# mit-acl/dpgo

Hardware: AMD Instinct MI355X
Metric: rbcd_iterations_per_sec (higher is better)
Workload: dtype f64; 1 GPU; synthetic 3-D grid 50x50x40 (100000 poses, 293500 edges), init = perturbed truth; agents=1, agents_per_gpu=1, r=5, d=3, schedule=single agent, poses_per_agent=100000, nnzb_per_agent=687000

## Files before the change

### dpgo_amd/csrc/agents.hip

```cpp
#include "host.h"

namespace dpgo_host {

int rebuild_vals(dpgo_problem_s* p, int nnzb, const int32_t* cptr, const int32_t* cedge, const uint8_t* ckind,
                 const double* base, double sign, double* out) {
  if (nnzb <= 0) return DPGO_OK;
  const int g = std::max(1, std::min(kMaxGrid, (nnzb + kBlock - 1) / kBlock));
  if (p->d == 2)
    launch(k_rebuild_Q<2>, g, 0, p->stream, p->gnc.dev(), cptr, cedge, ckind, base, sign, out, nnzb);
  else
    launch(k_rebuild_Q<3>, g, 0, p->stream, p->gnc.dev(), cptr, cedge, ckind, base, sign, out, nnzb);
  HIPC(hipGetLastError());
  return DPGO_OK;
}
int rebuild_Q_from_weights(dpgo_problem_s* p, const double* base, double sign, double* out) {
  return rebuild_vals(p, p->Q.nnzb, p->gnc.c_ptr, p->gnc.c_edge, p->gnc.c_kind, base, sign, out);
}
int rebuild_C_from_weights(dpgo_problem_s* p, const double* base, double sign, double* out) {
  if (!p->gnc.g_ptr) return DPGO_OK;
  return rebuild_vals(p, p->C.nnzb, p->gnc.g_ptr, p->gnc.g_edge, p->gnc.g_kind, base, sign, out);
}
int refresh_after_weights(dpgo_problem_s* p) {
  CHK(rebuild_Q_from_weights(p, p->gnc.q_base, 1.0, p->Q.vals));
  CHK(rebuild_C_from_weights(p, p->gnc.c_base, 1.0, p->C.vals));
// ... 633 lines not shown
  }
  HIPC(hipGetLastError());
  return DPGO_OK;
}
}
int dpgo_flags_wait_device(int n, unsigned long long* const* words_dev, const unsigned long long* values, int timeout_ms,
                           void* stream) {
  if (n < 0 || (n > 0 && (!words_dev || !values)) || timeout_ms <= 0) return fail(DPGO_ERR_INVALID, "bad ordering-word arguments");
  return flags_wait(n, words_dev, values, timeout_ms, nullptr, stream);
}
int dpgo_flags_wait_device_checked(int n, unsigned long long* const* words_dev, const unsigned long long* values,
                                   long long timeout_ms, unsigned long long* err_word, void* stream) {
  if (n < 0 || (n > 0 && (!words_dev || !values)) || timeout_ms < 0 || (timeout_ms > 0 && !err_word))
    return fail(DPGO_ERR_INVALID, "bad ordering-word arguments");
  return flags_wait(n, words_dev, values, timeout_ms, err_word, stream);
}

int dpgo_exchange_plan_destroy(dpgo_exchange_plan_t pl) {
  delete pl;
  return DPGO_OK;
}


int dpgo_max_translation_distance_device(int r, int d, int n, const double* X_dev, const double* Xprev_dev,
                                         double* out_dev, double* out_host, void* stream) {
  if (!X_dev || !Xprev_dev || !out_dev || n <= 0) return fail(DPGO_ERR_INVALID, "bad arguments");
  hipStream_t s = (hipStream_t)stream;
  HIPC(hipMemsetAsync(out_dev, 0, sizeof(double), s));
  const int g = std::max(1, std::min(kMaxGrid, (n + kBlock - 1) / kBlock));
  CHK(dispatch_dr(d, r, [&](auto D, auto R) {
    return launch(k_max_translation_distance<D, R>, g, 0, s, X_dev, Xprev_dev, n,
                  reinterpret_cast<unsigned long long*>(out_dev));
  }));
  HIPC(hipGetLastError());
  if (out_host) {
    HIPC(hipMemcpyAsync(out_host, out_dev, sizeof(double), hipMemcpyDeviceToHost, s));
    HIPC(hipStreamSynchronize(s));
  }
  return DPGO_OK;
}


int dpgo_manifold_project(int r, int d, int n, const double* M, double* out, int device) {
  if (!M || !out) return fail(DPGO_ERR_INVALID, "null pointer");
  CHK(manifold_args(r, d, n, device));
  const size_t total = (size_t)n * (d + 1) * r, vb = sizeof(double) * total;
  DevBuf<double> a, o;
  CHK(a.alloc(total));
  CHK(o.alloc(total));
  HIPC(hipMemcpy(a, M, vb, hipMemcpyHostToDevice));
  CHK(dpgo_manifold_project_device(r, d, n, a, o, nullptr));
  HIPC(hipMemcpy(out, o, vb, hipMemcpyDeviceToHost));
  return DPGO_OK;
}


int dpgo_manifold_tangent_project(int r, int d, int n, const double* X, const double* V, double* out, int device) {
  if (!X || !V || !out) return fail(DPGO_ERR_INVALID, "null pointer");
  CHK(manifold_args(r, d, n, device));
  const size_t total = (size_t)n * (d + 1) * r, vb = sizeof(double) * total;
  DevBuf<double> x, v, o;
  for (DevBuf<double>* q : {&x, &v, &o}) CHK(q->alloc(total));
  HIPC(hipMemcpy(x, X, vb, hipMemcpyHostToDevice));
  HIPC(hipMemcpy(v, V, vb, hipMemcpyHostToDevice));
  CHK(dispatch_dr(d, r, [&](auto D, auto R) {
    return launch(k_precond<D, R>, tiles_grid(d, n), 0, nullptr, x, v, nullptr, o, n);
  }));
  HIPC(hipGetLastError());
  HIPC(hipMemcpy(out, o, vb, hipMemcpyDeviceToHost));
  return DPGO_OK;
}


int dpgo_manifold_retract(int r, int d, int n, const double* X, const double* eta, double scale, double* out,
                          int device) {
  if (!X || !eta || !out) return fail(DPGO_ERR_INVALID, "null pointer");
  CHK(manifold_args(r, d, n, device));
  const size_t total = (size_t)n * (d + 1) * r, vb = sizeof(double) * total;
  DevBuf<double> x, v, o;
  for (DevBuf<double>* q : {&x, &v, &o}) CHK(q->alloc(total));
  HIPC(hipMemcpy(x, X, vb, hipMemcpyHostToDevice));
  HIPC(hipMemcpy(v, eta, vb, hipMemcpyHostToDevice));
  CHK(dispatch_dr(d, r, [&](auto D, auto R) {
    return launch(k_retract<D, R>, tiles_grid(d, n), 0, nullptr, x, v, scale, o, nullptr, n, nullptr, nullptr, nullptr);
  }));
  HIPC(hipGetLastError());
  HIPC(hipMemcpy(out, o, vb, hipMemcpyDeviceToHost));
  return DPGO_OK;
}

}
```

### dpgo_amd/csrc/host.h

```cpp
#pragma once
#include "kernels.h"

#include <algorithm>
#include <atomic>
#include <chrono>
#include <condition_variable>
#include <functional>
#include <memory>
#include <pthread.h>
#include <sched.h>
#include <mutex>
#include <thread>
#include <type_traits>
#include <cmath>
#include <cstdio>
#include <cstdlib>
#include <cstring>
#include <string>
#include <utility>
#include <vector>

#include "../../include/dpgo_hip.h"

using namespace dpgo;
// ... 76 lines not shown

template <class T, bool kPinned>
class OwnedBuf {
 public:
  OwnedBuf() = default;
  OwnedBuf(OwnedBuf&& o) noexcept : p_(std::exchange(o.p_, nullptr)), bytes_(std::exchange(o.bytes_, 0)) {}
  OwnedBuf& operator=(OwnedBuf&& o) noexcept {
    if (this != &o) {
      reset();
      p_ = std::exchange(o.p_, nullptr);
      bytes_ = std::exchange(o.bytes_, 0);
    }
    return *this;
  }
  ~OwnedBuf() { reset(); }
  int alloc(size_t count, unsigned flags = hipHostMallocDefault) {
    reset();
    const size_t bytes = sizeof(T) * count;
    if constexpr (kPinned)
      HIPC(hipHostMalloc(&p_, bytes, flags));
    else
      HIPC(hipMalloc(&p_, bytes));
    if (!p_) return DPGO_OK;
    bytes_ = bytes;
    g_live_buffers.fetch_add(1, std::memory_order_relaxed);
    g_live_bytes.fetch_add((long long)bytes, std::memory_order_relaxed);
    return DPGO_OK;
  }
  void reset() {
    if (!p_) return;
    if constexpr (kPinned)
      (void)hipHostFree(p_);
    else
      (void)hipFree(p_);
    g_live_buffers.fetch_sub(1, std::memory_order_relaxed);
    g_live_bytes.fetch_sub((long long)bytes_, std::memory_order_relaxed);
    p_ = nullptr;
    bytes_ = 0;
  }
  T* get() const { return p_; }
  operator T*() const { return p_; }
  T* operator->() const { return p_; }

 private:
  T* p_ = nullptr;
  size_t bytes_ = 0;
};
template <class T>
using DevBuf = OwnedBuf<T, false>;
template <class T>
using PinBuf = OwnedBuf<T, true>;

template <class T>
inline int upload(DevBuf<T>& dst, const T* src, size_t count, hipStream_t s) {
  CHK(dst.alloc(count > 0 ? count : 1));
  if (count > 0) HIPC(hipMemcpyAsync(dst, src, sizeof(T) * count, hipMemcpyHostToDevice, s));
  return DPGO_OK;
}

struct OwnedStream {
  hipStream_t s = nullptr;
  OwnedStream() = default;
  OwnedStream(const OwnedStream&) = delete;
  OwnedStream& operator=(const OwnedStream&) = delete;
  ~OwnedStream() {
    if (s) (void)hipStreamDestroy(s);
  }
  operator hipStream_t() const { return s; }
};

struct Bsr {
  int nrows = 0, ncols = 0, nnzb = 0;
  DevBuf<int32_t> rowptr, colidx;
  DevBuf<double> vals;
  BsrDev dev() const { return BsrDev{rowptr, colidx, vals}; }
};

#define DPGO_OPTIONS(X)                                                                                                  \
  X(split,             "DPGO_SPLIT",              0,  "lane groups per pose of the SpMM-family kernels: 1, 2, 4 (0: by size)")       \
  X(spmm_symmetric,    "DPGO_SPMM_SYMMETRIC",    -1,  "symmetric storage of Q for blocks beyond the Infinity Cache: 0 / 1")          \
  X(stream_nt,         "DPGO_STREAM_NT",         -1,  "non-temporal single-use operands in the tCG-step kernels: 0 / 1")             \
  X(outer_sym,         "DPGO_OUTER_SYM",          1,  "outer RTR iteration (k_grad / k_hess) reads the symmetric copy when tCG does") \
  X(rho_exact,         "DPGO_RHO_EXACT",          0,  "rho test from a fresh H eta (k_hess, one more pass over Q) instead of tCG's residual: reference path") \
  X(tile_walk,         "DPGO_TILE_WALK",          1,  "symmetric-storage kernels walk each XCD's tiles breadth-first over the tile graph (0: index order)") \
  X(tcg_ahead,         "DPGO_TCG_AHEAD",          0,  "iterations the just-in-time feed stays ahead (0: 2 multilevel / 4 otherwise)") \
  X(grid_update,       "DPGO_GRID_UPDATE",        0,  "launch cap of k_tcg_update (0: resident count)")                              \
  X(grid_hess,         "DPGO_GRID_HESS",          0,  "launch cap of k_tcg_hess (0: resident count)")                                \
  X(grid_hess_sym,     "DPGO_GRID_HESS_SYM",      0,  "launch cap of k_tcg_hess_sym (0: resident count)")                            \
  X(grid_retract,      "DPGO_GRID_RETRACT",       0,  "launch cap of k_retract (0: 1024)")                                           \
  X(grid_outer_sym,    "DPGO_GRID_OUTER_SYM",     0,  "launch cap of k_grad / k_hess on the symmetric storage (0: resident count)")  \
  X(grid_spmm_sym,     "DPGO_GRID_SPMM_SYM",      0,  "launch cap of k_spmm_sym (0: resident count, at most 1024)")                  \
  X(grid_ml,           "DPGO_GRID_ML",            0,  "launch cap of the level-0 restriction / post-smoothing (0: resident count)")  \
  X(grid_edges,        "DPGO_GRID_EDGES",         0,  "launch cap of k_edge_robust, GNC and robust re-weighting alike (0: 1024)")    \
  X(persist,           "DPGO_PERSIST",           -1,  "one-launch solve (k_rtr_persist) off / on whatever the size: 0 / 1")          \
  X(persist_max_poses, "DPGO_PERSIST_MAX_POSES",  0,  "largest block the one-launch solve takes (0: every block it can hold)")       \
  X(persist_split,     "DPGO_PERSIST_SPLIT",      0,  "lane groups per pose of the one-launch solve: 1, 4 (0: by size)")             \
  X(persist_mt,        "DPGO_PERSIST_MT",         0,  "tiles per workgroup of the one-launch solve: 1, 2 (0: by size)")              \
  X(additive_tiles,    "DPGO_ADDITIVE_TILES",     1,  "workgroup tiles per aggregate of the additive one-launch solve: 1, 2 (opt-in: blocks up to ~28 000 poses)") \
  X(poll_first,        "DPGO_POLL_FIRST",        -1,  "s_sleep units before the first sweep of the in-kernel all-reduce")            \
  X(poll_sleep,        "DPGO_POLL_SLEEP",        -1,  "s_sleep units between sweeps of the in-kernel all-reduce")                    \
  X(poll_first_pay,    "DPGO_POLL_FIRST_PAY",    -1,  "the same before the first sweep of a reduction that carries a payload")       \
  X(persist_verbose,   "DPGO_PERSIST_VERBOSE",    0,  "per-solve phase report of the one-launch solve on stderr")                    \
  X(setup_timing,      "DPGO_SETUP_TIMING",       0,  "section times of the hierarchy's symbolic set-up on stderr")                  \
  X(setup_threads,     "DPGO_SETUP_THREADS",      0,  "host threads of the hierarchy's symbolic set-up (0: min(8, cores); 1: serial)") \
  X(setup_pin,         "DPGO_SETUP_PIN",          1,  "set-up worker threads placed in the CPU group of the thread that first used them") \
  X(auto_cost_rule,    "DPGO_AUTO_COST_RULE",     1,  "DPGO_PRECOND_AUTO on coupled blocks: cost rule (0: tCG-budget hysteresis only)") \
  X(ml_graph,          "DPGO_ML_GRAPH",           1,  "graph aggregates in the default hierarchy (0: index runs)")                   \
  X(ml_graph_size,     "DPGO_ML_GRAPH_SIZE",      0,  "growth size of the default graph aggregates (0: by size)")                    \
  X(ml_growth_chunks,  "DPGO_ML_GROWTH_CHUNKS",   0,  "index ranges the graph aggregates grow and merge in (0: 8 from 65 536 poses, else 1)") \
  X(ml_ap,             "DPGO_ML_AP",              1,  "two-level post-smoothing through A P (0: gather through Q; index runs only)") \
  X(ml_dense_sym,      "DPGO_ML_DENSE_SYM",      -1,  "dense level from the packed lower triangle on the matrix cores: 0 / 1")       \
  X(ml_early_stop,     "DPGO_ML_EARLY_STOP",      1,  "tCG's residual test in the restriction kernel, one kernel early")             \
  X(ml_operator_bits,  "DPGO_ML_OPERATOR_BITS",   0,  "level-0 operator copies of the cycle on HBM-bound blocks: 32 / 64 (0: 32)")   \
  X(ml_vector_bits,    "DPGO_ML_VECTOR_BITS",     0,  "cycle-internal vectors (pre-smoothed iterate, kept residual) beside fp32 operator copies: 32 / 64 (0: 32)") \
  X(ml_dense_bits,     "DPGO_ML_DENSE_BITS",      0,  "dense level beside fp32 cycle vectors: 32 / 64 (0: 64 -- fp32 measured neutral)") \
  X(gj_mfma,           "DPGO_GJ_MFMA",            1,  "rank-64 updates of the dense inverse on the fp64 matrix cores")               \
  X(dense_chunk,       "DPGO_DENSE_CHUNK",        0,  "tiles per workgroup of k_dense_sym_apply (0: default)")                       \
  X(coarse_nodes,      "DPGO_COARSE_NODES",       0,  "nodes per workgroup of k_ml_coarse_prolong: 1-4 (0: by size)")                \
  X(coarse_grid,       "DPGO_COARSE_GRID",        0,  "launch cap of k_ml_coarse_prolong (0: default)")                              \
  X(coarse_nt,         "DPGO_COARSE_NT",         -1,  "non-temporal loads of the dense inverse: 0 / 1")
struct Options {
#define X(field, var, unset, text) int field = unset;
  DPGO_OPTIONS(X)
#undef X
};
inline Options& options_storage() {
  static Options o;
  return o;
}
inline void options_read(Options& o) {
  o = Options();
#define X(field, var, unset, text) \
  if (const char* e_ = std::getenv(var)) o.field = (*e_ == 0) ? 1 : std::atoi(e_);
  DPGO_OPTIONS(X)
#undef X
}
inline const Options& options() {
  static const bool once = (options_read(options_storage()), true);
  (void)once;
  return options_storage();
}
inline std::string options_describe() {
  const Options& o = options();
  std::string s;
#define X(field, var, unset, text) s += std::string(var) + "=" + std::to_string(o.field) + (o.field == (unset) ? "" : " [set]") + "  # " + text + "\n";
  DPGO_OPTIONS(X)
#undef X
  return s;
}

}
using namespace dpgo_host;

struct dpgo_problem_s {
  int r = 0, d = 0, n = 0, b = 0, T = 0;
  int device = 0;
  OwnedStream own_stream;
  hipStream_t stream = nullptr;
  Bsr Q;
  Bsr C;
  DevBuf<double> G0, G;
  bool has_G = false;
  DevBuf<double> dinv;
  double dinv_shift = -1.0;
  DevBuf<double> x1_buf, x2, g1, g2, eta, delta, Hd, rr, z, S1, S2;
  double* x1 = nullptr;
  struct MlLevel {
    int n = 0;
    int k = 0;
    int split = 1;
    Bsr A;
    DevBuf<int32_t> slot_row;
    DevBuf<double> dinv, Pb;
    DevBuf<double> r, x1, x;
    Bsr AP;
    DevBuf<double> res1;
    bool graph = false;
    DevBuf<int32_t> lab, agg_ptr, agg_mem, parent, pslot;
    DevBuf<int32_t> mem_pos;
    DevBuf<int32_t> seg_info, seg_ptr;
    int nseg = 0;
    DevBuf<int32_t> tile_perm;
    int perm_tile = 0;
    int merge_cap = 0;
    DevBuf<double> tbuf;
    DevBuf<float> Pb32, AP32;
    DevBuf<float> x1f, res1f;
    AggMap agg() const { return AggMap{graph ? lab : nullptr, k}; }
  };
  std::vector<MlLevel> ml;
  std::vector<int32_t> h_rowptr, h_colidx;
  bool ml_symbolic = false, ml_ready = false, ml_user_ks = false;
  bool ml_additive_layout = false;
  struct AddPlan {
    int split = 0, tile = 0, S = 0, cap = 0, na = 0;
    bool graph = true;
  } add_plan;
  bool add_plan_known = false;
  int add_tiles = 0;
  struct AggCache {
    int S = 0, cap = 0;
    std::vector<int32_t> lab, ptr, mem, parent, pslot;
  } add_agg;
  double ml_omega = 0.7, ml_shift = 1e-1;
  struct DenseLevel {
    DevBuf<double> inv;
    DevBuf<float> inv32;
    DevBuf<double> packed, pd, pt;
    DevBuf<DenseChunk> chunks;
    DevBuf<int> chunk_first;
    int nchunks = 0;
    int lda = 0;
    DevBuf<double> W, Rx;
  } dense;
  bool ml_use_dense_sym() const {
    const int env = options().ml_dense_sym;
    if (!ml_use_ap() || ml_coarse_bits != 64 || !dense.packed || env == 0) return false;
    return env == 1 || dense.lda >= 3072;
  }
  int ml_coarse_bits = 64;
  int ml_operator_bits = 32;
  bool ml_ops32_ready = false;
  bool ml_ops32_suspend = false;
  bool ml_ops32_wanted() const { return ml_operator_bits == 32 && tcg_sym && split == 1 && ml_use_ap() && sym.uvalsT != nullptr; }
  bool ml_ops32_active() const { return !ml_ops32_suspend && ml_ops32_wanted() && ml_ops32_ready; }
  bool ml_vec32_active() const { return ml_ops32_active() && options().ml_vector_bits != 64; }
  bool coarse32_active() const {
    return ml_coarse_bits == 32 || (ml_vec32_active() && !ml_use_dense_sym() && options().ml_dense_bits == 32);
  }
  bool auto_ml = false, auto_decided = false;
  struct AutoCost {
    long long jac_units = 0;
    int ref = 0;
    int state = 0;
    int backoff = 0;
    int switches = 0;
    int last_used = -1, last_products = 0;
    int uj = 10, ua = 18;
  } auto_cost;
  void auto_decide() {
    if (!auto_decided) {
      auto_ml = !(has_G || C.nnzb > 0);
      auto_decided = true;
      auto_cost = AutoCost();
    }
  }
  bool ml_use_ap() const {
    const bool off = options().ml_ap == 0;
    return ml.size() == 2 && ml[0].AP.vals != nullptr && (!off || ml[0].graph);
// ... 161 lines not shown
    wait(submit(count, fn, max_threads));
  }
  void warm(int threads) {
    bool expected = false;
    if (threads <= 1 || !warmed_.compare_exchange_strong(expected, true)) return;
    std::thread([this, threads] { wait(submit(threads - 1, [](int) {}, threads)); }).detach();
  }

 private:
  static constexpr int kMaxWorkers = 15;
  int home_cpu_ = -1;
  void pin(int) {
    if (!pin_enabled() || home_cpu_ < 0) return;
    cpu_set_t allowed, want;
    CPU_ZERO(&allowed);
    CPU_ZERO(&want);
    if (sched_getaffinity(0, sizeof(allowed), &allowed) != 0) return;
    const int lo = home_cpu_ & ~7;
    int cnt = 0;
    for (int c = lo; c < lo + 8; ++c)
      if (c < CPU_SETSIZE && CPU_ISSET(c, &allowed)) CPU_SET(c, &want), ++cnt;
    if (cnt >= 2) (void)pthread_setaffinity_np(pthread_self(), sizeof(want), &want);
  }
  static bool pin_enabled() { return options().setup_pin != 0; }
  TaskPool() { home_cpu_ = sched_getcpu(); }
  static void help(Batch& b) {
    for (;;) {
      const int k = b.next.fetch_add(1, std::memory_order_relaxed);
      if (k >= b.count) return;
      b.fn(k);
      b.done.fetch_add(1, std::memory_order_release);
    }
  }
  void loop() {
    for (;;) {
      Job b;
      {
        std::unique_lock<std::mutex> lk(mu_);
        cv_.wait(lk, [this] { return !queue_.empty(); });
        b = std::move(queue_.front());
        queue_.erase(queue_.begin());
      }
      help(*b);
    }
  }
  std::mutex mu_;
  std::condition_variable cv_;
  std::vector<Job> queue_;
  unsigned nworkers_ = 0;
  std::atomic<bool> warmed_{false};
};
struct JobGuard {
  TaskPool::Job job;
  ~JobGuard() { TaskPool::get().wait(job); }
};

struct PersistGeo {
  int split = 0, mt = 0, wgs = 0, slots = 0;
};

enum { RUN_FULL = 0, RUN_BEGIN = 1, RUN_END = 2 };

int set_device(dpgo_problem_s* p);
int upload_bsr(Bsr& m, int nrows, int ncols, int nnzb, int b, const int32_t* rowptr, const int32_t* colidx,
               const double* vals, hipStream_t s);
int validate_bsr(int nrows, int ncols, int nnzb, const int32_t* rowptr, const int32_t* colidx, bool need_diag);
int build_dinv(dpgo_problem_s* p, double shift);
int poll_state(dpgo_problem_s* p);
int push_state(dpgo_problem_s* p);
void sym_free(dpgo_problem_s* p);
int launch_spmm_view(dpgo_problem_s* p, const BsrDev& M, const double* V, const double* Gadd, double* OUT, int rows, int g,
                     bool stream_nt = false);
int sym_symbolic_setup(dpgo_problem_s* p);
int sym_ensure(dpgo_problem_s* p, bool* usable);
int launch_spmm_sym(dpgo_problem_s* p, const BsrSymDev& M, const double* V, const double* Gadd, double* OUT);
int launch_spmm(dpgo_problem_s* p, const Bsr& M, const double* V, const double* Gadd, double* OUT, int nrows = -1,
                bool plain_only = false);
bool outer_sym_enabled();
int launch_grad(dpgo_problem_s* p, const double* X, double* RG, double* S, double* EG,
                const DevState* st = nullptr, bool sym = false);
int launch_hess(dpgo_problem_s* p, const double* X, const double* S, const double* V, const double* Gdot,
                double* HV, double* partials, const DevState* st, int check_tcg, bool sym = false);
int launch_retract(dpgo_problem_s* p, const double* X, const double* eta, double scale, double* X2,
                   const DevState* st, const double* rho_r = nullptr, const double* rho_g = nullptr);
int launch_rtr_update(dpgo_problem_s* p);
int launch_precond(dpgo_problem_s* p, const double* X, const double* V, const double* dinv, double* Z);
int launch_rtr_begin(dpgo_problem_s* p, double tol, double Delta0, double Dmax, int max_inner, int tiny);
int check_ready(dpgo_problem_s* p);
int h2d(dpgo_problem_s* p, double* dst, const double* src);
int d2h(dpgo_problem_s* p, double* dst, const double* src);

int ml_tile(int b, int split);
int additive_tile(const dpgo_problem_s* p);
int ml_level_split(int n);
int ml_default_graph_size(int n, int b);
std::vector<int> ml_default_ks(int n, int b, int split0);
void ml_free(dpgo_problem_s* p);
int ml_graph_aggregates(const std::vector<int32_t>& rowptr, const std::vector<int32_t>& colidx, int n, int S,
                        std::vector<int32_t>& lab, std::vector<int32_t>& ptr, std::vector<int32_t>& mem,
                        std::vector<int32_t>& parent, std::vector<int32_t>& pslot);
int ml_merge_small_aggregates(const std::vector<int32_t>& rowptr, const std::vector<int32_t>& colidx, int n, int S, int cap,
                              std::vector<int32_t>& lab, std::vector<int32_t>& ptr, std::vector<int32_t>& mem,
                              std::vector<int32_t>& parent, std::vector<int32_t>& pslot);
int ml_symbolic_setup(dpgo_problem_s* p, const std::vector<int>& ks_in, int perm_tile = 0);
int setup_threads();
int flat_grid(size_t items);
bool gj_use_mfma();
int dense_spd_inverse(hipStream_t s, double* M, int lda, double* W, double* Rx, bool mfma);
int ml_numeric_setup(dpgo_problem_s* p);
std::vector<int> ml_current_ks(const dpgo_problem_s* p);
const dpgo_problem_s::AddPlan& additive_plan(dpgo_problem_s* p);
int additive_split_of(const dpgo_problem_s* p);
int additive_tiles(const dpgo_problem_s* p);
int additive_mt_of(const dpgo_problem_s* p);
int ml_ensure(dpgo_problem_s* p, double shift, bool additive = false);
int ml_ops32_ensure(dpgo_problem_s* p);
int persist_capacity(int device);
int launch_coarse_prolong(dpgo_problem_s* p, const dpgo_problem_s::MlLevel& L, const dpgo_problem_s::MlLevel& C,
                          const DevState* gate, double* xc_out = nullptr);
int launch_dense_sym(dpgo_problem_s* p, const dpgo_problem_s::MlLevel& C, const DevState* gate);
int launch_ml_restrict0(dpgo_problem_s* p, const double* r, const DevState* gate, int g0, bool stop_check = false);
int launch_ml_post_ap(dpgo_problem_s* p, const double* Xdev, const double* r, double* z, double* pout, const DevState* gate);
int launch_ml_tail(dpgo_problem_s* p, const double* Xdev, const double* r, double* z, double* pout,
                   const DevState* gate, bool stop_check = false);
int launch_ml_apply(dpgo_problem_s* p, const double* Xdev, const double* v, double* z);

int launch_tcg_update(dpgo_problem_s* p, const double* dinv, int first, double* z_out = nullptr,
                      double ml_omega = 0.0);
int launch_tcg_hess(dpgo_problem_s* p, int first);
int launch_tcg_hess_with(dpgo_problem_s* p, const DevState* sin, DevState* sout, int first, unsigned long long* hflag,
                         unsigned gen);
int resolve_tcg_storage(dpgo_problem_s* p);
int persist_capacity(int device);
bool persist_reserve(dpgo_problem_s* p, int slots, int limit);
void persist_release(dpgo_problem_s* p);
bool additive_available(dpgo_problem_s* p);
PersistGeo persist_geometry(const dpgo_problem_s* p, int free_slots, int share = 1, bool additive = false);
bool additive_lds_fits(const dpgo_problem_s* p, int split, int mt, int na);
int launch_rtr_persistent(dpgo_problem_s* p, const dpgo_ropt_params* prm, const double* dinv, bool* used, bool additive);
void persist_report(dpgo_problem_s* p);
int rtr_outer_iteration(dpgo_problem_s* p, const dpgo_ropt_params* prm, const double* dinv, Counters& cnt,
                        bool poll_at_end);
int auto_units_jacobi(dpgo_problem_s* p);
int auto_units_additive(dpgo_problem_s* p);
void auto_update(dpgo_problem_s* p, const dpgo_ropt_params* prm, int used, int products);
int run_optimize(dpgo_problem_s* p, const dpgo_ropt_params* prm, dpgo_ropt_result* res, int phase = RUN_FULL);
int tune_launch_caps(dpgo_problem_s* p);
int tune_persist(dpgo_problem_s* p);

int rebuild_vals(dpgo_problem_s* p, int nnzb, const int32_t* cptr, const int32_t* cedge, const uint8_t* ckind,
                 const double* base, double sign, double* out);
int rebuild_Q_from_weights(dpgo_problem_s* p, const double* base, double sign, double* out);
int rebuild_C_from_weights(dpgo_problem_s* p, const double* base, double sign, double* out);
int refresh_after_weights(dpgo_problem_s* p);

}
```

### dpgo_amd/csrc/kernels/manifold.h

```cpp
#pragma once

template <int D, int R>
__global__ __launch_bounds__(kBlock) void k_precond(const double* __restrict__ X, const double* __restrict__ V,
                                                    const double* __restrict__ dinv, double* __restrict__ Z,
                                                    int n) {
  using GEO = Geo<D, R>;
  __shared__ double sm[kWaves][3][GEO::G][GEO::T];
  const LaneId L = lane_id<D>();
  const int ntiles = (n + GEO::P - 1) / GEO::P;
  const TileIter ti_ = tile_iter(ntiles);
  for (int tile = ti_.first; tile < ti_.last; tile += ti_.step) {
    const int i = tile * GEO::P + L.wave * GEO::G + L.g;
    const bool ok = (L.g < GEO::G) && (i < n);
    const size_t off = (size_t)i * GEO::T + L.c * R;
    double* ys = ok ? &sm[L.wave][0][L.g][0] : nullptr;
    double* vs = ok ? &sm[L.wave][1][L.g][0] : nullptr;
    double* zs = ok ? &sm[L.wave][2][L.g][0] : nullptr;
    double v[R], x[R], z[R];
    if (ok) {
      load_col<R>(X + off, x);
      load_col<R>(V + off, v);
      store_col<R>(ys + L.c * R, x);
      store_col<R>(vs + L.c * R, v);
    }
    wave_sync();
    if (ok) {
      if (dinv) {
        jacobi_col<D, R>(vs, dinv + (size_t)i * GEO::BB + L.c * GEO::B, z);
      } else {
#pragma unroll
        for (int a = 0; a < R; ++a) z[a] = v[a];
      }
      store_col<R>(zs + L.c * R, z);
    }
    wave_sync();
    if (ok) {
      double out[R], s[D];
      proj_col<D, R>(ys, zs, L.c, z, out, s);
      store_col<R>(Z + off, out);
    }
    wave_sync();
  }
}

template <int D, int R, bool RHO = false>
__global__ __launch_bounds__(kBlock) void k_retract(const double* __restrict__ X, const double* __restrict__ eta,
                                                    double scale, double* __restrict__ X2,
                                                    const DevState* __restrict__ st, int n,
                                                    const double* __restrict__ r, const double* __restrict__ g,
                                                    double* __restrict__ partials) {
  using GEO = Geo<D, R>;
  __shared__ double sm[kWaves][GEO::G][GEO::T];
  __shared__ double red[kWaves * kNP];
  if (st && st->rtr_stop) return;
  const LaneId L = lane_id<D>();
  const int ntiles = (n + GEO::P - 1) / GEO::P;
  [[maybe_unused]] double part[2] = {0.0, 0.0};
  const TileIter ti_ = tile_iter(ntiles);
  for (int tile = ti_.first; tile < ti_.last; tile += ti_.step) {
    const int i = tile * GEO::P + L.wave * GEO::G + L.g;
    const bool ok = (L.g < GEO::G) && (i < n);
    const size_t off = (size_t)i * GEO::T + L.c * R;
    double* as = ok ? &sm[L.wave][L.g][0] : nullptr;
    double a[R];
    if (ok) {
      double x[R], e[R];
      load_col<R>(X + off, x);
      load_col<R>(eta + off, e);
      if constexpr (RHO) {
        double rc[R], gc[R];
        load_col<R>(r + off, rc);
        load_col<R>(g + off, gc);
#pragma unroll
        for (int k = 0; k < R; ++k) {
          part[0] = fma(e[k], rc[k] - gc[k], part[0]);
          part[1] = fma(e[k], gc[k], part[1]);
        }
      }
#pragma unroll
      for (int k = 0; k < R; ++k) a[k] = fma(scale, e[k], x[k]);
      store_col<R>(as + L.c * R, a);
    }
    wave_sync();
    if (ok) {
      qf_col<D, R>(as, L.c, a);
      store_col<R>(X2 + off, a);
    }
    wave_sync();
  }
  if constexpr (RHO) store_partials<2>(part, partials, red);
}

constexpr double kJacobiTol = 0x1p-50;
constexpr double kJacobiZero = 0x1p-600;
constexpr int kJacobiSweeps = 30;
template <int D, int N>
__device__ __forceinline__ void jacobi_columns(double (&a)[D][N], double (&V)[D][D]) {
  double mx = 0.0;
#pragma unroll
  for (int p = 0; p < D; ++p)
#pragma unroll
    for (int k = 0; k < N; ++k) mx = fmax(mx, fabs(a[p][k]));
  const int ex = (mx > 0.0 && mx < INFINITY) ? -ilogb(mx) : 0;
#pragma unroll
  for (int p = 0; p < D; ++p) {
#pragma unroll
    for (int k = 0; k < N; ++k) a[p][k] = ldexp(a[p][k], ex);
#pragma unroll
    for (int q = 0; q < D; ++q) V[p][q] = (p == q) ? 1.0 : 0.0;
  }
  for (int sweep = 0; sweep < kJacobiSweeps; ++sweep) {
    bool rotated = false;
#pragma unroll
    for (int p = 0; p < D; ++p)
#pragma unroll
      for (int q = p + 1; q < D; ++q) {
        double al = 0.0, be = 0.0, ga = 0.0;
#pragma unroll
        for (int k = 0; k < N; ++k) {
          al = fma(a[p][k], a[p][k], al);
          be = fma(a[q][k], a[q][k], be);
          ga = fma(a[p][k], a[q][k], ga);
        }
        if (al > kJacobiZero && be > kJacobiZero && fabs(ga) > kJacobiTol * (sqrt(al) * sqrt(be))) {
          rotated = true;
          const double zeta = (be - al) / (2.0 * ga);
          const double t = (zeta >= 0.0 ? 1.0 : -1.0) / (fabs(zeta) + sqrt(zeta * zeta + 1.0));
          const double cs = 1.0 / sqrt(t * t + 1.0), sn = t * cs;
#pragma unroll
          for (int k = 0; k < N; ++k) {
            const double x = a[p][k], y = a[q][k];
            a[p][k] = cs * x - sn * y;
            a[q][k] = sn * x + cs * y;
          }
#pragma unroll
          for (int k = 0; k < D; ++k) {
            const double x = V[k][p], y = V[k][q];
            V[k][p] = cs * x - sn * y;
            V[k][q] = sn * x + cs * y;
          }
        }
      }
    if (!rotated) break;
  }
}
template <int D, int N>
__device__ __forceinline__ void jacobi_inv_norms(const double (&a)[D][N], double (&nrm2)[D], double (&inv)[D]) {
#pragma unroll
  for (int p = 0; p < D; ++p) {
    double s = 0.0;
#pragma unroll
// ... 143 lines not shown
```

### dpgo_amd/csrc/kernels/tcg.h

```cpp
#pragma once

__device__ __forceinline__ bool tcg_hess_prologue(DevState& st, const double* __restrict__ pin, int nb_in, int first,
                                                  double* red, double& beta, const PartialRaw<2>* early = nullptr) {
  double pr[2];
  if (early)
    partials_finish<2>(*early, pr, red);
  else
    load_partials<2>(pin, nb_in, pr, red);
  const double r_r = pr[0], z_r_new = pr[1];
  beta = 0.0;
  if (first) {
    st.norm_r0 = sqrt(r_r);
    st.z_r = z_r_new;
    st.d_Pd = z_r_new;
    st.e_Pd = 0.0;
    if (st.max_inner <= 0) {
      st.tcg_done = 1;
      return false;
    }
    return true;
  }
  const double norm_r = sqrt(r_r);
  const double pw = (st.theta == 1.0) ? st.norm_r0 : pow(st.norm_r0, st.theta);
  if (st.tcg_j >= st.min_inner && norm_r <= st.norm_r0 * (pw < st.kappa ? pw : st.kappa)) {
    st.tcg_status = (st.kappa < pw) ? TCG_LCON : TCG_SCON;
    st.tcg_done = 1;
    return false;
  }
  beta = z_r_new / st.z_r;
  st.e_Pd = beta * (st.e_Pd + st.alpha * st.d_Pd);
  st.d_Pd = z_r_new + beta * beta * st.d_Pd;
  st.z_r = z_r_new;
  st.tcg_j += 1;
  if (st.tcg_j >= st.max_inner) {
    st.tcg_done = 1;
    st.tcg_status = TCG_MAXITER;
    return false;
  }
  return true;
}

__device__ __forceinline__ int tcg_update_prologue(DevState& st, const double* __restrict__ pin, int nb_in, int first,
                                                   double* red, double& alpha, double& tau,
                                                   const PartialRaw<1>* early = nullptr) {
  alpha = 0.0;
  tau = 0.0;
  if (first) {
    st.tcg_done = 0;
    st.tcg_j = 0;
    st.tcg_status = TCG_MAXITER;
    st.e_Pe = 0.0;
    st.e_Pd = 0.0;
    return 2;
  }
  double dh[1];
  if (early)
    partials_finish<1>(*early, dh, red);
  else
    load_partials<1>(pin, nb_in, dh, red);
  const double d_Hd = dh[0];
  alpha = st.z_r / d_Hd;
  const double e_Pe_new = st.e_Pe + 2.0 * alpha * st.e_Pd + alpha * alpha * st.d_Pd;
  st.n_hess += 1;
  st.alpha = alpha;
  const double D2 = st.Delta * st.Delta;
  if (d_Hd <= 0.0 || e_Pe_new >= D2) {
    tau = (-st.e_Pd + sqrt(st.e_Pd * st.e_Pd + st.d_Pd * (D2 - st.e_Pe))) / st.d_Pd;
    st.tcg_status = (d_Hd < 0.0) ? TCG_NEGCURV : TCG_EXCREGION;
    st.tcg_done = 1;
    return 1;
  }
  st.e_Pe = e_Pe_new;
  return 0;
}

template <int D, int R, int SPLIT>
__global__ __launch_bounds__(kBlock, DPGO_LB_HESS) void k_tcg_hess(BsrDev Q, const double* __restrict__ X,
                                                     const double* __restrict__ S, const double* __restrict__ z,
                                                     double* __restrict__ delta, double* __restrict__ Hd,
                                                     const double* __restrict__ pin, int nb_in,
                                                     double* __restrict__ pout, const DevState* __restrict__ sin,
                                                     DevState* __restrict__ sout, int first, int n,
                                                     unsigned long long* hflag, unsigned gen) {
  using GEO = Geo<D, R, SPLIT>;
  __shared__ __attribute__((aligned(16))) double sm[kWaves][3][GEO::G][GEO::T];
  __shared__ double red[kWaves * kNP];
  DevState st;
  load_state(st, sin);
  gen = state_gen(st, gen);
  if (st.rtr_stop || st.tcg_done) {
    if (blockIdx.x == 0 && threadIdx.x == 0) {
      store_state(sout, st);
      publish_progress(hflag, gen, st);
    }
    return;
  }
  double beta;
  const bool go = tcg_hess_prologue(st, pin, nb_in, first, red, beta);
  if (blockIdx.x == 0 && threadIdx.x == 0) {
    store_state(sout, st);
    publish_progress(hflag, gen, st);
  }
  if (!go) return;

  const LaneId L = lane_id<D, SPLIT>();
  const int ntiles = (n + GEO::P - 1) / GEO::P;
  double part[1] = {0.0};
  const TileIter ti_ = tile_iter(ntiles);
  for (int tile = ti_.first; tile < ti_.last; tile += ti_.step) {
    const int i = tile * GEO::P + L.wave * GEO::G + L.g;
    const bool okp = (L.g < GEO::G) && (i < n);
    const bool ok = okp && (L.s == 0);
    double h[R], zc[R], x[R];
    const size_t off = (size_t)i * GEO::T + L.c * R;
    double* ys = ok ? &sm[L.wave][0][L.g][0] : nullptr;
    double* vs = ok ? &sm[L.wave][1][L.g][0] : nullptr;
    double* hs = ok ? &sm[L.wave][2][L.g][0] : nullptr;
    double srow[D], dl[R], hd[R];
    if (ok) {
      load_col<R>(X + off, x);
      load_col<R>(z + off, zc);
      if (L.c < D) {
#pragma unroll
        for (int a = 0; a < D; ++a) srow[a] = S[(size_t)i * D * D + L.c * D + a];
      }
      if (!first) {
        load_col<R>(delta + off, dl);
        load_col<R>(Hd + off, hd);
      }
    }
    spmm_col<D, R, SPLIT>(Q.rowptr, Q.colidx, Q.vals, z, i, L.s, L.c, okp, h);
    if (ok) {
      store_col<R>(ys + L.c * R, x);
      store_col<R>(vs + L.c * R, zc);
    }
    wave_sync();
    if (ok) {
      if (L.c < D) {
#pragma unroll
        for (int a = 0; a < D; ++a) {
#pragma unroll
          for (int k = 0; k < R; ++k) h[k] = fma(-vs[a * R + k], srow[a], h[k]);
        }
      }
      store_col<R>(hs + L.c * R, h);
    }
    wave_sync();
    if (ok) {
      double hz[R], s[D];
      proj_col<D, R>(ys, hs, L.c, h, hz, s);
      if (first) {
#pragma unroll
        for (int a = 0; a < R; ++a) {
          dl[a] = -zc[a];
          hd[a] = -hz[a];
        }
      } else {
#pragma unroll
        for (int a = 0; a < R; ++a) {
          dl[a] = fma(beta, dl[a], -zc[a]);
          hd[a] = fma(beta, hd[a], -hz[a]);
        }
      }
#pragma unroll
      for (int a = 0; a < R; ++a) part[0] = fma(dl[a], hd[a], part[0]);
      store_col<R>(delta + off, dl);
      store_col<R>(Hd + off, hd);
    }
    wave_sync();
  }
  store_partials<1>(part, pout, red);
}

template <int D, int R, int SPLIT, int NTS = 0>
__global__ __launch_bounds__(kBlock) void k_tcg_hess_span(BsrDev Q, const double* __restrict__ X,
                                                          const double* __restrict__ S, const double* __restrict__ z,
                                                          double* __restrict__ delta, double* __restrict__ Hd,
                                                          const double* __restrict__ pin, int nb_in,
                                                          double* __restrict__ pout, const DevState* __restrict__ sin,
                                                          DevState* __restrict__ sout, int first, int n,
                                                          unsigned long long* hflag, unsigned gen) {
  using GEO = Geo<D, R, SPLIT>;
  using SPN = Span<D, R, SPLIT>;
  __shared__ __attribute__((aligned(16))) double sm[kWaves][4][GEO::G][GEO::T];
  __shared__ double red[kWaves * kNP];
  const LaneId L = lane_id<D, SPLIT>();
  const int lane = threadIdx.x & 63;
  const int ntiles = (n + GEO::P - 1) / GEO::P;
  const TileIter ti_ = tile_iter(ntiles);
  double* ys = &sm[L.wave][0][0][0];
  double* vs = &sm[L.wave][1][0][0];
  double* hs = &sm[L.wave][2][0][0];
  double* os = &sm[L.wave][3][0][0];

  RowIdx ri;
  dbl2 xv[SPN::NIT], zv[SPN::NIT], dv[SPN::NIT], hv[SPN::NIT];
  double srow[D];
  int p0 = 0, valid = 0, i = 0;
  bool okp = false, ok = false;
  auto prefetch = [&](int tile) {
    p0 = tile * GEO::P + L.wave * GEO::G;
    const int npose = (n - p0) < GEO::G ? (n - p0) : GEO::G;
    valid = npose > 0 ? npose * GEO::T : 0;
    i = p0 + L.g;
    okp = (L.g < GEO::G) && (i < n);
    ok = okp && (L.s == 0);
    ri = row_idx_load<D, SPLIT>(Q.rowptr, Q.colidx, i, L.s, L.c, okp);
    const size_t base = (size_t)p0 * GEO::T;
    const dbl2* X2 = reinterpret_cast<const dbl2*>(X + base);
    const dbl2* z2 = reinterpret_cast<const dbl2*>(z + base);
    const dbl2* d2 = reinterpret_cast<const dbl2*>(delta + base);
    const dbl2* h2 = reinterpret_cast<const dbl2*>(Hd + base);
#pragma unroll
    for (int it = 0; it < SPN::NIT; ++it) {
      const int pc = lane + 64 * it;
      if (2 * pc < valid) {
        xv[it] = ld_stream<NTS>(X2 + pc);
        zv[it] = z2[pc];
        if (!first) {
          dv[it] = ld_stream<NTS>(d2 + pc);
          hv[it] = ld_stream<NTS>(h2 + pc);
        }
      }
    }
    if (ok && L.c < D) {
#pragma unroll
      for (int a = 0; a < D; ++a) srow[a] = ld_stream<NTS>(S + (size_t)i * D * D + L.c * D + a);
    }
  };
  DPGO_TL_DECL;
  DPGO_STAMP(0, 0);
  DevState st;
  load_state(st, sin);
  gen = state_gen(st, gen);
  [[maybe_unused]] PartialRaw<2> praw;
  if constexpr (SPLIT > 1) partials_issue<2>(pin, nb_in, praw);
  int tile = ti_.first;
  bool have = tile < ti_.last;
  if (have) prefetch(tile);

  DPGO_STAMP(0, 1);
  if (st.rtr_stop || st.tcg_done) {
    if (blockIdx.x == 0 && threadIdx.x == 0) {
      store_state(sout, st);
      publish_progress(hflag, gen, st);
    }
    return;
  }
  double beta;
  const bool go = tcg_hess_prologue(st, pin, nb_in, first, red, beta, (SPLIT > 1) ? &praw : nullptr);
  if (blockIdx.x == 0 && threadIdx.x == 0) {
    store_state(sout, st);
    publish_progress(hflag, gen, st);
  }
  if (!go) return;
  DPGO_STAMP(0, 2);

  double part[1] = {0.0};
  while (have) {
#pragma unroll
    for (int it = 0; it < SPN::NIT; ++it) {
      const int pc = lane + 64 * it;
      if (2 * pc < valid) {
        reinterpret_cast<dbl2*>(ys)[pc] = xv[it];
        reinterpret_cast<dbl2*>(vs)[pc] = zv[it];
      }
    }
    DPGO_STAMP(0, 3);
    double h[R];
    spmm_col_pre<D, R, SPLIT>(ri, Q.colidx, Q.vals, z, L.s, L.c, h);
    wave_sync();
    DPGO_STAMP(0, 4);
    if (ok) {
      if (L.c < D) {
        const double* vt = vs + L.g * GEO::T;
#pragma unroll
        for (int a = 0; a < D; ++a) {
#pragma unroll
          for (int k = 0; k < R; ++k) h[k] = fma(-vt[a * R + k], srow[a], h[k]);
        }
      }
      store_col<R>(hs + L.g * GEO::T + L.c * R, h);
    }
    wave_sync();
    if (ok) {
      double hz[R], sdummy[D];
      proj_col<D, R>(ys + L.g * GEO::T, hs + L.g * GEO::T, L.c, h, hz, sdummy);
      store_col<R>(os + L.g * GEO::T + L.c * R, hz);
    }
    wave_sync();
    {
      const size_t base = (size_t)p0 * GEO::T;
      dbl2* d2 = reinterpret_cast<dbl2*>(delta + base);
      dbl2* h2 = reinterpret_cast<dbl2*>(Hd + base);
#pragma unroll
      for (int it = 0; it < SPN::NIT; ++it) {
        const int pc = lane + 64 * it;
        if (2 * pc < valid) {
          const dbl2 hzv = reinterpret_cast<const dbl2*>(os)[pc];
          dbl2 dn, hn;
          if (first) {
            dn.x = -zv[it].x;
            dn.y = -zv[it].y;
            hn.x = -hzv.x;
            hn.y = -hzv.y;
          } else {
            dn.x = fma(beta, dv[it].x, -zv[it].x);
            dn.y = fma(beta, dv[it].y, -zv[it].y);
            hn.x = fma(beta, hv[it].x, -hzv.x);
            hn.y = fma(beta, hv[it].y, -hzv.y);
          }
          st_stream<NTS>(d2 + pc, dn);
          st_stream<NTS>(h2 + pc, hn);
          part[0] = fma(dn.x, hn.x, part[0]);
          part[0] = fma(dn.y, hn.y, part[0]);
        }
      }
    }
    wave_sync();
    DPGO_STAMP(0, 5);
    tile += ti_.step;
    have = tile < ti_.last;
    if (have) prefetch(tile);
  }
  store_partials<1>(part, pout, red);
  DPGO_STAMP(0, 6);
  DPGO_COMMIT(0);
}

template <int D, int R, int NTS>
__global__ __launch_bounds__(kBlock) __attribute__((amdgpu_waves_per_eu(DPGO_SYM_WAVES, DPGO_SYM_WAVES))) void k_tcg_hess_sym(BsrSymDev Q, const double* __restrict__ X,
                                                          const double* __restrict__ S, const double* __restrict__ z,
                                                          double* __restrict__ delta, double* __restrict__ Hd,
                                                          const double* __restrict__ pin, int nb_in,
                                                          double* __restrict__ pout, const DevState* __restrict__ sin,
                                                          DevState* __restrict__ sout, int first, int n,
                                                          unsigned long long* hflag, unsigned gen) {
  constexpr int SPLIT = 1;
  using GEO = Geo<D, R, SPLIT>;
  using SPN = Span<D, R, SPLIT>;
  __shared__ __attribute__((aligned(16))) double sm[kWaves][4][GEO::G][GEO::T];
  __shared__ double red[kWaves * kNP];
  const LaneId L = lane_id<D, SPLIT>();
  const int lane = threadIdx.x & 63;
  const int ntiles = (n + GEO::P - 1) / GEO::P;
  const TileIter ti_ = tile_iter(ntiles);
  double* ys = &sm[L.wave][0][0][0];
  double* vs = &sm[L.wave][1][0][0];
  double* hs = &sm[L.wave][2][0][0];
  double* os = &sm[L.wave][3][0][0];

  SymIdx si;
  dbl2 xv[SPN::NIT], zv[SPN::NIT];
  double srow[D];
  int p0 = 0, valid = 0, i = 0;
  bool okp = false, ok = false;
  auto prefetch = [&](int tk) {
    const int tile = tile_of(Q, tk);
    p0 = tile * GEO::P + L.wave * GEO::G;
    const int npose = (n - p0) < GEO::G ? (n - p0) : GEO::G;
    valid = npose > 0 ? npose * GEO::T : 0;
    i = p0 + L.g;
    okp = (L.g < GEO::G) && (i < n);
    ok = okp && (L.s == 0);
    si = sym_idx_load<D>(Q, i, L.c, okp);
    const size_t base = (size_t)p0 * GEO::T;
    const dbl2* X2 = reinterpret_cast<const dbl2*>(X + base);
    const dbl2* z2 = reinterpret_cast<const dbl2*>(z + base);
#pragma unroll
    for (int it = 0; it < SPN::NIT; ++it) {
      const int pc = lane + 64 * it;
      if (2 * pc < valid) {
        xv[it] = ld_stream<NTS>(X2 + pc);
        zv[it] = z2[pc];
      }
    }
    if (ok && L.c < D) {
#pragma unroll
      for (int a = 0; a < D; ++a) srow[a] = ld_stream<NTS>(S + (size_t)i * D * D + L.c * D + a);
    }
  };
  DPGO_TL_DECL;
  DPGO_TL_TILES_DECL;
  DPGO_STAMP(0, 0);
  DevState st;
  load_state(st, sin);
  gen = state_gen(st, gen);
  [[maybe_unused]] PartialRaw<2> praw;
  int tile = ti_.first;
  bool have = tile < ti_.last;
  if (have) prefetch(tile);

  DPGO_STAMP(0, 1);
  if (st.rtr_stop || st.tcg_done) {
    if (blockIdx.x == 0 && threadIdx.x == 0) {
      store_state(sout, st);
      publish_progress(hflag, gen, st);
    }
    return;
  }
  double beta;
  const bool go = tcg_hess_prologue(st, pin, nb_in, first, red, beta, (SPLIT > 1) ? &praw : nullptr);
  if (blockIdx.x == 0 && threadIdx.x == 0) {
    store_state(sout, st);
    publish_progress(hflag, gen, st);
  }
  if (!go) return;
  DPGO_STAMP(0, 2);
  DPGO_STAMP_ENTRY;
  DPGO_STAMP_AT(1);

  double part[1] = {0.0};
  while (have) {
    DPGO_STAMP_TILE(0);
#pragma unroll
    for (int it = 0; it < SPN::NIT; ++it) {
      const int pc = lane + 64 * it;
      if (2 * pc < valid) {
        reinterpret_cast<dbl2*>(ys)[pc] = xv[it];
        reinterpret_cast<dbl2*>(vs)[pc] = zv[it];
      }
    }
    DPGO_STAMP(0, 3);
    DPGO_STAMP_TILE(1);
    double h[R];
    spmm_sym_pre<D, R, DPGO_HESS_BATCH>(si, Q, z, L.c, h);
    DPGO_TL_USE(h[0]);
    DPGO_STAMP_TILE(2);
    dbl2 dv[SPN::NIT], hv[SPN::NIT];
    if (!first) {
      const size_t base = (size_t)p0 * GEO::T;
      const dbl2* d2 = reinterpret_cast<const dbl2*>(delta + base);
      const dbl2* h2 = reinterpret_cast<const dbl2*>(Hd + base);
#pragma unroll
      for (int it = 0; it < SPN::NIT; ++it) {
        const int pc = lane + 64 * it;
        if (2 * pc < valid) {
          dv[it] = ld_stream<NTS>(d2 + pc);
          hv[it] = ld_stream<NTS>(h2 + pc);
        }
      }
    }
    wave_sync();
    DPGO_STAMP(0, 4);
    DPGO_STAMP_TILE(3);
    if (ok) {
      if (L.c < D) {
        const double* vt = vs + L.g * GEO::T;
#pragma unroll
        for (int a = 0; a < D; ++a) {
#pragma unroll
          for (int k = 0; k < R; ++k) h[k] = fma(-vt[a * R + k], srow[a], h[k]);
        }
      }
      store_col<R>(hs + L.g * GEO::T + L.c * R, h);
    }
    wave_sync();
    if (ok) {
      double hz[R], sdummy[D];
      proj_col<D, R>(ys + L.g * GEO::T, hs + L.g * GEO::T, L.c, h, hz, sdummy);
      store_col<R>(os + L.g * GEO::T + L.c * R, hz);
    }
    wave_sync();
    DPGO_STAMP_TILE(4);
    {
      const size_t base = (size_t)p0 * GEO::T;
      dbl2* d2 = reinterpret_cast<dbl2*>(delta + base);
      dbl2* h2 = reinterpret_cast<dbl2*>(Hd + base);
#pragma unroll
      for (int it = 0; it < SPN::NIT; ++it) {
        const int pc = lane + 64 * it;
        if (2 * pc < valid) {
          const dbl2 hzv = reinterpret_cast<const dbl2*>(os)[pc];
          const dbl2 zl = reinterpret_cast<const dbl2*>(vs)[pc];
          dbl2 dn, hn;
          if (first) {
            dn.x = -zl.x;
            dn.y = -zl.y;
            hn.x = -hzv.x;
            hn.y = -hzv.y;
          } else {
            dn.x = fma(beta, dv[it].x, -zl.x);
            dn.y = fma(beta, dv[it].y, -zl.y);
            hn.x = fma(beta, hv[it].x, -hzv.x);
            hn.y = fma(beta, hv[it].y, -hzv.y);
          }
          st_stream<NTS>(d2 + pc, dn);
          st_stream<NTS>(h2 + pc, hn);
          part[0] = fma(dn.x, hn.x, part[0]);
          part[0] = fma(dn.y, hn.y, part[0]);
        }
      }
    }
    wave_sync();
    DPGO_STAMP(0, 5);
    tile += ti_.step;
    have = tile < ti_.last;
    if (have) prefetch(tile);
    DPGO_STAMP_TILE(5);
    DPGO_TILE_NEXT;
  }
  store_partials<1>(part, pout, red);
  DPGO_STAMP(0, 6);
  DPGO_STAMP_AT(2);
  DPGO_COMMIT(0);
}

#ifndef DPGO_UPDATE_WAVES
#define DPGO_UPDATE_WAVES 0
#endif
#ifndef DPGO_UPDATE_WAVES_ML
#define DPGO_UPDATE_WAVES_ML 3
#endif
template <int D, int R, int ML = 0>
__global__ __launch_bounds__(kBlock)
    __attribute__((amdgpu_waves_per_eu(ML ? DPGO_UPDATE_WAVES_ML : (DPGO_UPDATE_WAVES ? DPGO_UPDATE_WAVES : 1),
                                       ML ? DPGO_UPDATE_WAVES_ML : (DPGO_UPDATE_WAVES ? DPGO_UPDATE_WAVES : 8))))
void k_tcg_update_span(const double* __restrict__ X, const double* __restrict__ g,
                                                            const double* __restrict__ dinv,
                                                            const double* __restrict__ delta,
                                                            const double* __restrict__ Hd, double* __restrict__ eta,
                                                            double* __restrict__ r, double* __restrict__ z,
                                                            const double* __restrict__ pin, int nb_in,
                                                            double* __restrict__ pout, const DevState* __restrict__ sin,
                                                            DevState* __restrict__ sout, int first, int n,
                                                            unsigned long long* hflag, unsigned gen,
                                                            double ml_omega, float* __restrict__ z32 = nullptr) {
  using GEO = Geo<D, R>;
  using SPN = Span<D, R, 1>;
  __shared__ __attribute__((aligned(16))) double sm[kWaves][4][GEO::G][GEO::T];
  __shared__ double red[kWaves * kNP];
  const LaneId L = lane_id<D>();
  const int lane = threadIdx.x & 63;
  const int ntiles = (n + GEO::P - 1) / GEO::P;
  const TileIter ti_ = tile_iter(ntiles);
  double* ys = &sm[L.wave][0][0][0];
  double* rs = &sm[L.wave][1][0][0];
  double* zs = &sm[L.wave][2][0][0];
  double* os = &sm[L.wave][3][0][0];

  const bool ml_mode = ML ? true : (ml_omega > 0.0);
  dbl2 xv[SPN::NIT], ev[SPN::NIT], dv[SPN::NIT], hv[SPN::NIT], rv[SPN::NIT];
  double drow[GEO::B];
  int p0 = 0, valid = 0, i = 0;
  bool ok = false;
  auto prefetch = [&](int tile) {
    p0 = tile * GEO::P + L.wave * GEO::G;
    const int npose = (n - p0) < GEO::G ? (n - p0) : GEO::G;
    valid = npose > 0 ? npose * GEO::T : 0;
    i = p0 + L.g;
    ok = (L.g < GEO::G) && (i < n);
    const size_t base = (size_t)p0 * GEO::T;
    const dbl2* X2 = reinterpret_cast<const dbl2*>(X + base);
    const dbl2* g2 = reinterpret_cast<const dbl2*>(g + base);
    const dbl2* e2 = reinterpret_cast<const dbl2*>(eta + base);
    const dbl2* d2 = reinterpret_cast<const dbl2*>(delta + base);
    const dbl2* h2 = reinterpret_cast<const dbl2*>(Hd + base);
    const dbl2* r2 = reinterpret_cast<const dbl2*>(r + base);
#pragma unroll
    for (int it = 0; it < SPN::NIT; ++it) {
      const int pc = lane + 64 * it;
      if (2 * pc < valid) {
        if (!ml_mode) xv[it] = X2[pc];
        if (first) {
          rv[it] = g2[pc];
        } else {
          ev[it] = e2[pc];
          dv[it] = d2[pc];
          hv[it] = h2[pc];
          rv[it] = r2[pc];
        }
      }
    }
    if (ok && dinv) {
#pragma unroll
      for (int k = 0; k < GEO::B; ++k) drow[k] = dinv[(size_t)i * GEO::BB + L.c * GEO::B + k];
    }
  };
  DPGO_TL_DECL;
  DPGO_STAMP(1, 0);
  DevState st;
  load_state(st, sin);
  gen = state_gen(st, gen);
  PartialRaw<1> praw;
  partials_issue<1>(pin, nb_in, praw);
  int tile = ti_.first;
  bool have = tile < ti_.last;
  if (have) prefetch(tile);

  if (st.rtr_stop || (!first && st.tcg_done)) {
    if (blockIdx.x == 0 && threadIdx.x == 0) {
      store_state(sout, st);
      publish_progress(hflag, gen, st);
    }
    return;
  }
  double alpha, tau;
  const int mode = tcg_update_prologue(st, pin, nb_in, first, red, alpha, tau, &praw);
  if (blockIdx.x == 0 && threadIdx.x == 0) {
    store_state(sout, st);
    publish_progress(hflag, gen, st);
  }

  DPGO_STAMP(1, 2);
  double part[2] = {0.0, 0.0};
  while (have) {
    const size_t base = (size_t)p0 * GEO::T;
    dbl2* eta2 = reinterpret_cast<dbl2*>(eta + base);
    if (mode == 1) {
      dbl2* r2 = reinterpret_cast<dbl2*>(r + base);
#pragma unroll
      for (int it = 0; it < SPN::NIT; ++it) {
        const int pc = lane + 64 * it;
        if (2 * pc < valid) {
          dbl2 e = ev[it], rr = rv[it];
          e.x = fma(tau, dv[it].x, e.x);
          e.y = fma(tau, dv[it].y, e.y);
          rr.x = fma(tau, hv[it].x, rr.x);
          rr.y = fma(tau, hv[it].y, rr.y);
          eta2[pc] = e;
          r2[pc] = rr;
        }
      }
    } else {
      dbl2* r2 = reinterpret_cast<dbl2*>(r + base);
#pragma unroll
      for (int it = 0; it < SPN::NIT; ++it) {
        const int pc = lane + 64 * it;
        if (2 * pc < valid) {
          if (!ml_mode) reinterpret_cast<dbl2*>(ys)[pc] = xv[it];
          dbl2 rr = rv[it];
          if (mode == 2) {
            dbl2 zero;
            zero.x = 0.0;
            zero.y = 0.0;
            eta2[pc] = zero;
          } else {
            dbl2 e = ev[it];
            e.x = fma(alpha, dv[it].x, e.x);
            e.y = fma(alpha, dv[it].y, e.y);
            rr.x = fma(alpha, hv[it].x, rr.x);
            rr.y = fma(alpha, hv[it].y, rr.y);
            eta2[pc] = e;
          }
          r2[pc] = rr;
          reinterpret_cast<dbl2*>(rs)[pc] = rr;
          part[0] = fma(rr.x, rr.x, part[0]);
          part[0] = fma(rr.y, rr.y, part[0]);
        }
      }
      wave_sync();
      double zz[R];
      if (ok) {
        const double* rt = rs + L.g * GEO::T;
        if (dinv) {
          jacobi_col<D, R>(rt, drow, zz);
        } else {
#pragma unroll
          for (int a = 0; a < R; ++a) zz[a] = rt[L.c * R + a];
        }
        store_col<R>(zs + L.g * GEO::T + L.c * R, zz);
      }
      wave_sync();
      if (ok) {
        double out[R], sdummy[D];
        if (ml_mode) {
#pragma unroll
          for (int a = 0; a < R; ++a) out[a] = ml_omega * zz[a];
        } else {
          proj_col<D, R>(ys + L.g * GEO::T, zs + L.g * GEO::T, L.c, zz, out, sdummy);
        }
        const double* rt = rs + L.g * GEO::T + L.c * R;
#pragma unroll
        for (int a = 0; a < R; ++a) part[1] = fma(out[a], rt[a], part[1]);
        store_col<R>(os + L.g * GEO::T + L.c * R, out);
      }
      wave_sync();
      if (z32) {
        float2* zf = reinterpret_cast<float2*>(z32 + base);
#pragma unroll
        for (int it = 0; it < SPN::NIT; ++it) {
          const int pc = lane + 64 * it;
          if (2 * pc < valid) {
            const dbl2 v = reinterpret_cast<const dbl2*>(os)[pc];
            zf[pc] = make_float2((float)v.x, (float)v.y);
          }
        }
      } else {
        dbl2* z2 = reinterpret_cast<dbl2*>(z + base);
#pragma unroll
        for (int it = 0; it < SPN::NIT; ++it) {
          const int pc = lane + 64 * it;
          if (2 * pc < valid) z2[pc] = reinterpret_cast<const dbl2*>(os)[pc];
        }
      }
      wave_sync();
    }
    DPGO_STAMP(1, 5);
    tile += ti_.step;
    have = tile < ti_.last;
    if (have) prefetch(tile);
  }
  if (mode != 1) store_partials<2>(part, pout, red);
  DPGO_STAMP(1, 6);
  DPGO_COMMIT(1);
}

template <int D, int R>
__global__ __launch_bounds__(kBlock, DPGO_LB_UPDATE) void k_tcg_update(const double* __restrict__ X, const double* __restrict__ g,
                                                       const double* __restrict__ dinv,
                                                       const double* __restrict__ delta,
                                                       const double* __restrict__ Hd, double* __restrict__ eta,
                                                       double* __restrict__ r, double* __restrict__ z,
                                                       const double* __restrict__ pin, int nb_in,
                                                       double* __restrict__ pout, const DevState* __restrict__ sin,
                                                       DevState* __restrict__ sout, int first, int n,
                                                       unsigned long long* hflag, unsigned gen, double ml_omega) {
  using GEO = Geo<D, R>;
  __shared__ __attribute__((aligned(16))) double sm[kWaves][3][GEO::G][GEO::T];
  __shared__ double red[kWaves * kNP];
  DevState st;
  load_state(st, sin);
  gen = state_gen(st, gen);
  if (st.rtr_stop || (!first && st.tcg_done)) {
    if (blockIdx.x == 0 && threadIdx.x == 0) {
      store_state(sout, st);
      publish_progress(hflag, gen, st);
    }
    return;
  }
  double alpha, tau;
  const int mode = tcg_update_prologue(st, pin, nb_in, first, red, alpha, tau);
  if (blockIdx.x == 0 && threadIdx.x == 0) {
    store_state(sout, st);
    publish_progress(hflag, gen, st);
  }

  const LaneId L = lane_id<D>();
  const int ntiles = (n + GEO::P - 1) / GEO::P;
  double part[2] = {0.0, 0.0};
  const TileIter ti_ = tile_iter(ntiles);
  for (int tile = ti_.first; tile < ti_.last; tile += ti_.step) {
    const int i = tile * GEO::P + L.wave * GEO::G + L.g;
    const bool ok = (L.g < GEO::G) && (i < n);
    const size_t off = (size_t)i * GEO::T + L.c * R;
    if (mode == 1) {
      if (ok) {
        double e[R], dl[R], hd[R], rr[R];
        load_col<R>(eta + off, e);
        load_col<R>(delta + off, dl);
        load_col<R>(Hd + off, hd);
        load_col<R>(r + off, rr);
#pragma unroll
        for (int a = 0; a < R; ++a) {
          e[a] = fma(tau, dl[a], e[a]);
          rr[a] = fma(tau, hd[a], rr[a]);
        }
        store_col<R>(eta + off, e);
        store_col<R>(r + off, rr);
      }
      continue;
    }
    double* ys = ok ? &sm[L.wave][0][L.g][0] : nullptr;
    double* rs = ok ? &sm[L.wave][1][L.g][0] : nullptr;
    double* zs = ok ? &sm[L.wave][2][L.g][0] : nullptr;
    double rr[R], x[R], zz[R], drow[GEO::B];
    if (ok) {
      load_col<R>(X + off, x);
      if (dinv) {
#pragma unroll
        for (int k = 0; k < GEO::B; ++k) drow[k] = dinv[(size_t)i * GEO::BB + L.c * GEO::B + k];
      }
      if (mode == 2) {
        load_col<R>(g + off, rr);
        double e[R];
#pragma unroll
        for (int a = 0; a < R; ++a) e[a] = 0.0;
        store_col<R>(eta + off, e);
      } else {
        double e[R], dl[R], hd[R];
        load_col<R>(eta + off, e);
        load_col<R>(delta + off, dl);
        load_col<R>(Hd + off, hd);
        load_col<R>(r + off, rr);
#pragma unroll
        for (int a = 0; a < R; ++a) {
          e[a] = fma(alpha, dl[a], e[a]);
          rr[a] = fma(alpha, hd[a], rr[a]);
        }
        store_col<R>(eta + off, e);
      }
      store_col<R>(r + off, rr);
#pragma unroll
      for (int a = 0; a < R; ++a) part[0] = fma(rr[a], rr[a], part[0]);
      store_col<R>(ys + L.c * R, x);
      store_col<R>(rs + L.c * R, rr);
    }
    wave_sync();
    if (ok) {
      if (dinv) {
        jacobi_col<D, R>(rs, drow, zz);
      } else {
#pragma unroll
        for (int a = 0; a < R; ++a) zz[a] = rr[a];
      }
      store_col<R>(zs + L.c * R, zz);
    }
    wave_sync();
    if (ok) {
      double out[R], s[D];
      if (ml_omega > 0.0) {
#pragma unroll
        for (int a = 0; a < R; ++a) out[a] = ml_omega * zz[a];
      } else {
        proj_col<D, R>(ys, zs, L.c, zz, out, s);
      }
#pragma unroll
      for (int a = 0; a < R; ++a) part[1] = fma(out[a], rr[a], part[1]);
      store_col<R>(z + off, out);
    }
    wave_sync();
  }
  if (mode != 1) store_partials<2>(part, pout, red);
}
```

### dpgo_amd/csrc/problem.hip

```cpp
#include "host.h"

namespace dpgo_host {

int set_device(dpgo_problem_s* p) {
  HIPC(hipSetDevice(p->device));
  return DPGO_OK;
}

int upload_bsr(Bsr& m, int nrows, int ncols, int nnzb, int b, const int32_t* rowptr, const int32_t* colidx,
               const double* vals, hipStream_t s) {
  m = Bsr();
  m.nrows = nrows;
  m.ncols = ncols;
  m.nnzb = nnzb;
  CHK(m.rowptr.alloc(nrows + 1));
  CHK(m.colidx.alloc(nnzb > 0 ? nnzb : 1));
  CHK(m.vals.alloc((size_t)(nnzb > 0 ? nnzb : 1) * b * b));
  HIPC(hipMemcpyAsync(m.rowptr, rowptr, sizeof(int32_t) * (nrows + 1), hipMemcpyHostToDevice, s));
  if (nnzb > 0) {
    HIPC(hipMemcpyAsync(m.colidx, colidx, sizeof(int32_t) * nnzb, hipMemcpyHostToDevice, s));
    if (vals) HIPC(hipMemcpyAsync(m.vals, vals, sizeof(double) * (size_t)nnzb * b * b, hipMemcpyHostToDevice, s));
  }
  HIPC(hipStreamSynchronize(s));
  return DPGO_OK;
// ... 149 lines not shown
    const int g = (int)std::min<size_t>(kMaxGrid, (total + kBlock - 1) / kBlock);
    HIPC(hipMemsetAsync(S.flag, 0, sizeof(int), p->stream));
    if (p->d == 2) {
      launch(k_sym_refresh<2>, g, 0, p->stream, p->Q.vals, S.usrc, S.uvalsT, S.nu);
      launch(k_sym_check<2>, g, 0, p->stream, p->Q.vals, S.lsrc, S.lslot, S.uvalsT, S.nl, S.flag);
    } else {
      launch(k_sym_refresh<3>, g, 0, p->stream, p->Q.vals, S.usrc, S.uvalsT, S.nu);
      launch(k_sym_check<3>, g, 0, p->stream, p->Q.vals, S.lsrc, S.lslot, S.uvalsT, S.nl, S.flag);
    }
    HIPC(hipGetLastError());
    int bad = 0;
    HIPC(hipMemcpyAsync(&bad, S.flag, sizeof(int), hipMemcpyDeviceToHost, p->stream));
    HIPC(hipStreamSynchronize(p->stream));
    S.values_ok = (bad == 0);
    S.ready = true;
    p->ml_ops32_ready = false;
  }
  *usable = S.values_ok;
  return DPGO_OK;
}

int launch_spmm_sym(dpgo_problem_s* p, const BsrSymDev& M, const double* V, const double* Gadd, double* OUT) {
  const int g = p->grid_spmm_sym();
  CHK(dispatch_dr(p->d, p->r, [&](auto D, auto R) {
    return launch(p->want_stream_nt() ? k_spmm_sym<D, R, 1> : k_spmm_sym<D, R, 0>, g, 0, p->stream, M, V, Gadd, OUT, p->n);
  }));
  HIPC(hipGetLastError());
  return DPGO_OK;
}

int launch_spmm_view(dpgo_problem_s* p, const BsrDev& M, const double* V, const double* Gadd, double* OUT, int rows, int g,
                     bool stream_nt) {
  CHK(dispatch_drs(p->d, p->r, p->split, [&](auto D, auto R, auto SPLIT) {
    if (stream_nt) return launch(k_spmm<D, R, 1, 1>, g, 0, p->stream, M, V, Gadd, OUT, rows);
    return launch(k_spmm<D, R, SPLIT>, g, 0, p->stream, M, V, Gadd, OUT, rows);
  }));
  HIPC(hipGetLastError());
  return DPGO_OK;
}

int launch_spmm(dpgo_problem_s* p, const Bsr& M, const double* V, const double* Gadd, double* OUT, int nrows, bool plain_only) {
  if (&M == &p->Q && nrows < 0 && !plain_only && p->sym_wanted()) {
    bool usable = false;
    CHK(sym_ensure(p, &usable));
    if (usable) return launch_spmm_sym(p, p->sym.dev(), V, Gadd, OUT);
  }
  const int rows = nrows >= 0 ? nrows : p->n;
  int g = p->grid_spmm();
  if (nrows >= 0) g = std::min(kMaxGrid, pose_tiles(rows, p->b, p->split));
  return launch_spmm_view(p, M.dev(), V, Gadd, OUT, rows, g, p->want_stream_nt() && p->split == 1 && &M == &p->Q);
}

bool outer_sym_enabled() {
  return options().outer_sym != 0;
}
int launch_grad(dpgo_problem_s* p, const double* X, double* RG, double* S, double* EG,
                const DevState* st, bool sym) {
  const double* Gm = p->has_G ? p->G : nullptr;
  sym = sym && p->split == 1;
  p->nb_grad = sym ? p->grid_outer_sym() : p->grid_s();
  CHK(dispatch_drs(p->d, p->r, p->split, [&](auto D, auto R, auto SPLIT) {
    if (sym) return launch(k_grad<D, R, 1, BsrSymDev>, p->nb_grad, 0, p->stream, p->sym.dev(), X, Gm, RG, S, EG, p->pE(), st, p->n);
    return launch(k_grad<D, R, SPLIT>, p->nb_grad, 0, p->stream, p->Q.dev(), X, Gm, RG, S, EG, p->pE(), st, p->n);
  }));
  HIPC(hipGetLastError());
  return DPGO_OK;
}

int launch_hess(dpgo_problem_s* p, const double* X, const double* S, const double* V, const double* Gdot,
                double* HV, double* partials, const DevState* st, int check_tcg, bool sym) {
  sym = sym && p->split == 1;
  p->nb_hess = sym ? p->grid_outer_sym() : p->grid_s();
  CHK(dispatch_drs(p->d, p->r, p->split, [&](auto D, auto R, auto SPLIT) {
    if (sym)
      return launch(k_hess<D, R, 1, BsrSymDev>, p->nb_hess, 0, p->stream, p->sym.dev(), X, S, V, Gdot, HV, partials, st,
                    check_tcg, p->n);
    return launch(k_hess<D, R, SPLIT>, p->nb_hess, 0, p->stream, p->Q.dev(), X, S, V, Gdot, HV, partials, st, check_tcg, p->n);
  }));
  HIPC(hipGetLastError());
  return DPGO_OK;
}

int launch_retract(dpgo_problem_s* p, const double* X, const double* eta, double scale, double* X2,
                   const DevState* st, const double* rho_r, const double* rho_g) {
  int gr = std::min(pose_tiles(p->n, p->b), options().grid_retract > 0 ? options().grid_retract : kMaxGrid);
  const bool rho = rho_r && rho_g;
  if (rho) {
    if (scale != 1.0) return fail(DPGO_ERR_STATE, "the rho-test sums of k_retract belong to the full step (scale 1)");
    gr = std::min(gr, kPartialCap);
    p->nb_hess = gr;
  }
  CHK(dispatch_dr(p->d, p->r, [&](auto D, auto R) {
    if (rho) return launch(k_retract<D, R, true>, gr, 0, p->stream, X, eta, scale, X2, st, p->n, rho_r, rho_g, p->pH());
    return launch(k_retract<D, R, false>, gr, 0, p->stream, X, eta, scale, X2, st, p->n, nullptr, nullptr, nullptr);
  }));
  HIPC(hipGetLastError());
  return DPGO_OK;
}

int launch_rtr_update(dpgo_problem_s* p) {
  const int ge = p->nb_grad > 0 ? p->nb_grad : p->grid_s(), gh = p->nb_hess > 0 ? p->nb_hess : p->grid_s();
  CHK(dispatch_dr(p->d, p->r, [&](auto D, auto R) {
    return launch(k_rtr_update<D, R>, p->grid_flat(), 0, p->stream, p->x1, p->x2, p->g1, p->g2, p->S1, p->S2, p->pE(), ge,
                  p->pH(), gh, p->dstate + p->cur, p->dstate + (p->cur ^ 1), p->n);
  }));
  HIPC(hipGetLastError());
  p->cur ^= 1;
  std::swap(p->g1, p->g2);
  std::swap(p->S1, p->S2);
  return DPGO_OK;
}

int launch_precond(dpgo_problem_s* p, const double* X, const double* V, const double* dinv, double* Z) {
  CHK(dispatch_dr(p->d, p->r, [&](auto D, auto R) {
    return launch(k_precond<D, R>, p->grid(), 0, p->stream, X, V, dinv, Z, p->n);
  }));
  HIPC(hipGetLastError());
  return DPGO_OK;
}

int launch_rtr_begin(dpgo_problem_s* p, double tol, double Delta0, double Dmax, int max_inner, int tiny) {
  launch(k_rtr_begin, 1, 0, p->stream, p->pE(), p->nb_grad > 0 ? p->nb_grad : p->grid_s(), p->dstate, tol, Delta0, Dmax,
         max_inner, tiny);
  HIPC(hipGetLastError());
  p->cur = 0;
  return DPGO_OK;
}

int check_ready(dpgo_problem_s* p) {
  if (!p) return fail(DPGO_ERR_INVALID, "null handle");
  if (!p->Q.vals) return fail(DPGO_ERR_STATE, "quadratic matrix Q not set");
  return set_device(p);
}

int h2d(dpgo_problem_s* p, double* dst, const double* src) {
  HIPC(hipMemcpyAsync(dst, src, p->vec_bytes(), hipMemcpyHostToDevice, p->stream));
  return DPGO_OK;
}
int d2h(dpgo_problem_s* p, double* dst, const double* src) {
  HIPC(hipMemcpyAsync(dst, src, p->vec_bytes(), hipMemcpyDeviceToHost, p->stream));
  HIPC(hipStreamSynchronize(p->stream));
  return DPGO_OK;
}

}

extern "C" {


const char* dpgo_version(void) { return "dpgo_hip 0.1 (gfx950)"; }
const char* dpgo_last_error(void) { return g_err.c_str(); }
void dpgo_set_last_error(const char* msg) { g_err = msg ? msg : ""; }

int dpgo_device_count(int* count) {
  if (!count) return fail(DPGO_ERR_INVALID, "null count");
  int c = 0;
  hipError_t e = hipGetDeviceCount(&c);
  if (e != hipSuccess) {
    *count = 0;
    return fail(DPGO_ERR_HIP, std::string("hipGetDeviceCount: ") + hipGetErrorString(e));
  }
  *count = c;
  return DPGO_OK;
}


void dpgo_ropt_params_default(dpgo_ropt_params* p) {
  if (!p) return;
  p->method = DPGO_METHOD_RTR;
  p->verbose = 0;
  p->gradnorm_tol = 1e-2;
  p->RGD_stepsize = 1e-3;
  p->RGD_use_preconditioner = 1;
  p->RTR_iterations = 3;
  p->RTR_tCG_iterations = 50;
  p->RTR_initial_radius = 100.0;
  p->precond = DPGO_PRECOND_AUTO;
// ... 83 lines not shown
  std::string s = "dpgo_hip problem: d=" + std::to_string(p->d) + " r=" + std::to_string(p->r) + " n=" + std::to_string(p->n) +
                  " nnzb=" + std::to_string(p->Q.nnzb) + " device=" + std::to_string(p->device) + "\n";
  s += "  lane groups per pose " + std::to_string(p->split) + "; launch caps update/hess/hess_sym/restrict/post " +
       std::to_string(p->cap_u) + "/" + std::to_string(p->cap_h) + "/" + std::to_string(p->cap_hs) + "/" +
       std::to_string(p->cap_restrict) + "/" + std::to_string(p->cap_post) + "\n";
  s += std::string("  tCG-step storage: ") + (p->tcg_sym ? "symmetric" : "plain") + (p->stream_nt ? ", non-temporal single-use operands" : "") +
       "; coupling " + ((p->has_G || p->C.nnzb > 0) ? "yes" : "no") + "\n";
  s += std::string("  one-launch solve: ") + ((p->persist && !p->persist_failed_once) ? "on" : "off") + ", last geometry " +
       std::to_string(p->persist_wgs) + " workgroups x " + std::to_string(p->persist_split) + " lane groups x " +
       std::to_string(p->persist_mt) + " tiles" + (p->persist_add ? " (additive)" : "") + "\n";
  s += std::string("  auto: ") + (p->auto_decided ? (p->auto_ml ? "multilevel" : "block-Jacobi") : "undecided") + ", cost-rule state " +
       std::to_string(p->auto_cost.state) + ", block-Jacobi units " + std::to_string(p->auto_cost.jac_units) + ", switches " +
       std::to_string(p->auto_cost.switches) + ", hand-backs " + std::to_string(p->auto_cost.backoff) + "\n";
  s += "  hierarchy:";
  if (!p->ml_symbolic) s += " none";
  for (size_t l = 0; l < p->ml.size(); ++l)
    s += " [" + std::to_string(p->ml[l].n) + " nodes" + (p->ml[l].k ? ", k=" + std::to_string(p->ml[l].graph ? -p->ml[l].k : p->ml[l].k) : ", dense") + "]";
  s += std::string(p->ml_ready ? " built" : " not built") + ", dense level fp" + std::to_string(p->coarse32_active() ? 32 : 64) +
       (p->ml_additive_layout ? ", additive layout" : "") + ", level-0 operator copies of the cycle fp" +
       std::to_string(p->ml_operator_bits) + (p->ml_ops32_active() ? " (in use)" : "") + "\n";
  s += "options:\n" + options_describe();
  return copy_text(s, out, capacity);
}

int dpgo_problem_destroy(dpgo_problem_t p) {
  if (!p) return DPGO_OK;
  (void)hipSetDevice(p->device);
  if (p->own_stream) (void)hipStreamSynchronize(p->own_stream);
  delete p;
  return DPGO_OK;
}


int dpgo_problem_set_stream(dpgo_problem_t p, void* hip_stream) {
  if (!p) return fail(DPGO_ERR_INVALID, "null handle");
  CHK(set_device(p));
  HIPC(hipStreamSynchronize(p->stream));
  p->stream = (hipStream_t)hip_stream;
  return DPGO_OK;
}


int dpgo_problem_use_own_stream(dpgo_problem_t p) {
  if (!p) return fail(DPGO_ERR_INVALID, "null handle");
  CHK(set_device(p));
  HIPC(hipStreamSynchronize(p->stream));
  p->stream = p->own_stream;
  return DPGO_OK;
}


int dpgo_problem_dims(dpgo_problem_t p, int* r, int* d, int* n, int* nnzb) {
  if (!p) return fail(DPGO_ERR_INVALID, "null handle");
  if (r) *r = p->r;
  if (d) *d = p->d;
  if (n) *n = p->n;
  if (nnzb) *nnzb = p->Q.nnzb;
  return DPGO_OK;
}


int dpgo_problem_set_Q_bsr(dpgo_problem_t p, int nnzb, const int32_t* rowptr, const int32_t* colidx,
                           const double* vals) {
  if (!p) return fail(DPGO_ERR_INVALID, "null handle");
  if (!vals) return fail(DPGO_ERR_INVALID, "null vals");
  CHK(validate_bsr(p->n, p->n, nnzb, rowptr, colidx, true));
  CHK(set_device(p));
  if (p->gnc.e_w) p->gnc = dpgo_problem_s::GncEdges();
  CHK(upload_bsr(p->Q, p->n, p->n, nnzb, p->b, rowptr, colidx, vals, p->stream));
  const bool same_pattern = (int)p->h_rowptr.size() == p->n + 1 && (int)p->h_colidx.size() == nnzb &&
                            std::equal(rowptr, rowptr + p->n + 1, p->h_rowptr.begin()) &&
                            std::equal(colidx, colidx + nnzb, p->h_colidx.begin());
  if (!same_pattern) {
    p->h_rowptr.assign(rowptr, rowptr + p->n + 1);
    p->h_colidx.assign(colidx, colidx + nnzb);
    p->add_plan_known = false;
    if (p->ml_user_ks && p->ml_symbolic) {
      const int perm_tile = p->ml[0].perm_tile;
      CHK(ml_symbolic_setup(p, ml_current_ks(p), perm_tile));
    } else {
      ml_free(p);
    }
    sym_free(p);
  }
  p->sym.ready = p->tcg_sym = false;
  p->ml_ready = false;
  p->auto_decided = false;
  p->dinv_shift = -1.0;
  CHK(build_dinv(p, 1e-1));
  HIPC(hipStreamSynchronize(p->stream));
  return DPGO_OK;
}


int dpgo_problem_set_Q_csr(dpgo_problem_t p, const int32_t* outer, const int32_t* inner, const double* values) {
  if (!p) return fail(DPGO_ERR_INVALID, "null handle");
  if (!outer || !inner || !values) return fail(DPGO_ERR_INVALID, "null CSR arrays");
  const int b = p->b, n = p->n;
  std::vector<int32_t> rowptr(n + 1, 0), colidx;
  std::vector<double> vals;
  std::vector<int> slot(n, -1);
  for (int i = 0; i < n; ++i) {
    const int first = (int)colidx.size();
    std::vector<int> cols;
    for (int rr = 0; rr < b; ++rr) {
      const int row = i * b + rr;
      if (outer[row + 1] < outer[row]) return fail(DPGO_ERR_INVALID, "CSR outer index not monotone");
      for (int t = outer[row]; t < outer[row + 1]; ++t) {
        const int c = inner[t];
        if (c < 0 || c >= n * b) return fail(DPGO_ERR_INVALID, "CSR column index out of range");
        const int j = c / b;
        if (slot[j] < 0) {
          slot[j] = 1;
          cols.push_back(j);
        }
      }
    }
    std::sort(cols.begin(), cols.end());
    for (size_t k = 0; k < cols.size(); ++k) slot[cols[k]] = first + (int)k;
    colidx.insert(colidx.end(), cols.begin(), cols.end());
    vals.resize(colidx.size() * (size_t)b * b, 0.0);
    for (int rr = 0; rr < b; ++rr) {
      const int row = i * b + rr;
      for (int t = outer[row]; t < outer[row + 1]; ++t) {
        const int c = inner[t];
        vals[(size_t)slot[c / b] * b * b + rr * b + (c % b)] += values[t];
      }
    }
    for (int j : cols) slot[j] = -1;
    rowptr[i + 1] = (int32_t)colidx.size();
  }
  return dpgo_problem_set_Q_bsr(p, (int)colidx.size(), rowptr.data(), colidx.data(), vals.data());
}


int dpgo_problem_update_Q_values(dpgo_problem_t p, const double* vals) {
  CHK(check_ready(p));
  if (!vals) return fail(DPGO_ERR_INVALID, "null vals");
  HIPC(hipMemcpyAsync(p->Q.vals, vals, sizeof(double) * (size_t)p->Q.nnzb * p->b * p->b, hipMemcpyHostToDevice,
                      p->stream));
  if (p->gnc.e_w) CHK(rebuild_Q_from_weights(p, p->Q.vals, -1.0, p->gnc.q_base));
  const double s = p->dinv_shift > 0 ? p->dinv_shift : 1e-1;
  p->dinv_shift = -1.0;
  p->ml_ready = false;
  p->auto_decided = false;
  p->sym.ready = p->tcg_sym = false;
  CHK(build_dinv(p, s));
  HIPC(hipStreamSynchronize(p->stream));
  return DPGO_OK;
}


int dpgo_problem_get_Q_values(dpgo_problem_t p, double* vals_host) {
  CHK(check_ready(p));
  if (!vals_host) return fail(DPGO_ERR_INVALID, "null vals");
  HIPC(hipMemcpyAsync(vals_host, p->Q.vals, sizeof(double) * (size_t)p->Q.nnzb * p->b * p->b, hipMemcpyDeviceToHost,
                      p->stream));
  HIPC(hipStreamSynchronize(p->stream));
  return DPGO_OK;
}


int dpgo_problem_set_G(dpgo_problem_t p, const double* G_host) {
  if (!p) return fail(DPGO_ERR_INVALID, "null handle");
  CHK(set_device(p));
  if (!G_host) {
// ... 241 lines not shown
```

### dpgo_amd/csrc/solve.hip

```cpp
#include "host.h"

namespace dpgo_host {

int launch_tcg_update(dpgo_problem_s* p, const double* dinv, int first, double* z_out,
                      double ml_omega) {
  const bool ml_mode = ml_omega > 0.0;
  const int g = p->grid_u(ml_mode);
  double* zt = z_out ? z_out : p->z;
  float* z32 = (ml_omega > 0.0 && !p->ml.empty() && z_out == p->ml[0].x1 && p->ml_vec32_active()) ? p->ml[0].x1f : nullptr;
  CHK(dispatch_dr(p->d, p->r, [&](auto Dc, auto Rc) {
    constexpr int D = decltype(Dc)::value, R = decltype(Rc)::value;
    auto go = [&](auto kernel, auto... z32_arg) {
      return launch(kernel, g, 0, p->stream, p->x1, p->g1, dinv, p->delta, p->Hd, p->eta, p->rr, zt, p->pA(), p->grid_s(),
                    p->pB(), p->dstate + p->cur, p->dstate + (p->cur ^ 1), first, p->n, p->hflag, p->gen, ml_omega,
                    z32_arg...);
    };
    if constexpr (Span<D, R, 1>::kOk) {
      return go(ml_mode ? k_tcg_update_span<D, R, 1> : k_tcg_update_span<D, R, 0>, z32);
    } else {
      if (z32) return fail(DPGO_ERR_STATE, "fp32 cycle vectors need the span kernels (even pose tile size)");
      return go(k_tcg_update<D, R>);
    }
  }));
  HIPC(hipGetLastError());
  p->cur ^= 1;
  return DPGO_OK;
}

template <int D, int R, class F>
int dispatch_tcg_hess(const dpgo_problem_s* p, F&& f) {
  if constexpr (Span<D, R, 1>::kOk) {
    if (p->tcg_sym) return f(p->stream_nt ? k_tcg_hess_sym<D, R, 1> : k_tcg_hess_sym<D, R, 0>, p->sym.dev());
    if (p->stream_nt && p->split == 1) return f(k_tcg_hess_span<D, R, 1, 1>, p->Q.dev());
    return dispatch_split(p->split, [&](auto Sc) { return f(k_tcg_hess_span<D, R, decltype(Sc)::value>, p->Q.dev()); });
  } else {
    return dispatch_split(p->split, [&](auto Sc) { return f(k_tcg_hess<D, R, decltype(Sc)::value>, p->Q.dev()); });
  }
}

int launch_tcg_hess_with(dpgo_problem_s* p, const DevState* sin, DevState* sout, int first, unsigned long long* hflag,
                         unsigned gen) {
  CHK(dispatch_dr(p->d, p->r, [&](auto Dc, auto Rc) {
    constexpr int D = decltype(Dc)::value, R = decltype(Rc)::value;
    return dispatch_tcg_hess<D, R>(p, [&](auto kernel, const auto& Q) {
      return launch(kernel, p->grid_s(), 0, p->stream, Q, p->x1, p->S1, p->z, p->delta, p->Hd, p->pB(), p->nb_zr(), p->pA(),
                    sin, sout, first, p->n, hflag, gen);
    });
  }));
  HIPC(hipGetLastError());
  return DPGO_OK;
}
int launch_tcg_hess(dpgo_problem_s* p, int first) {
  CHK(launch_tcg_hess_with(p, p->dstate + p->cur, p->dstate + (p->cur ^ 1), first, p->hflag, p->gen));
  p->cur ^= 1;
  return DPGO_OK;
}

static bool span_ok(int d, int r) {
  bool ok = false;
  (void)dispatch_dr(d, r, [&](auto Dc, auto Rc) {
    ok = Span<decltype(Dc)::value, decltype(Rc)::value, 1>::kOk;
    return DPGO_OK;
  });
  return ok;
}

int resolve_tcg_storage(dpgo_problem_s* p) {
  p->tcg_sym = false;
  p->stream_nt = p->want_stream_nt();
  if (!span_ok(p->d, p->r) || !p->sym_wanted()) return DPGO_OK;
  bool usable = false;
  CHK(sym_ensure(p, &usable));
  p->tcg_sym = usable;
  return DPGO_OK;
}

constexpr int kMaxDevices = 64;
std::atomic<int> g_warnings{0};
std::atomic<int> g_persist_used[kMaxDevices];
std::atomic<int> g_persist_cap[kMaxDevices];

int persist_capacity(int device) {
  int cap = g_persist_cap[device % kMaxDevices].load();
  if (cap == 0) {
    int cus = 0;
    if (hipDeviceGetAttribute(&cus, hipDeviceAttributeMultiprocessorCount, device) != hipSuccess || cus <= 0) cus = 1;
    cap = 2 * cus;
    g_persist_cap[device % kMaxDevices].store(cap);
  }
  return cap;
}
bool persist_reserve(dpgo_problem_s* p, int slots, int limit) {
  auto& used = g_persist_used[p->device % kMaxDevices];
  int cur = used.load();
  while (cur + slots <= limit)
    if (used.compare_exchange_weak(cur, cur + slots)) {
      p->persist_reserved = slots;
      return true;
    }
  return false;
}
void persist_release(dpgo_problem_s* p) {
  if (p->persist_reserved > 0) g_persist_used[p->device % kMaxDevices].fetch_sub(p->persist_reserved);
  p->persist_reserved = 0;
}

bool additive_available(dpgo_problem_s* p) {
  return p->persist && !p->persist_failed_once && additive_plan(p).split != 0;
}
template <class F>
int dispatch_persist(int split, int mt, bool additive, F&& f) {
  if (additive) {
    if (split == 4) return f(Int<4>{}, Int<1>{}, std::true_type{});
    return mt == 2 ? f(Int<1>{}, Int<2>{}, std::true_type{}) : f(Int<1>{}, Int<1>{}, std::true_type{});
  }
  if (split == 4) return mt == 1 ? f(Int<4>{}, Int<1>{}, std::false_type{}) : f(Int<4>{}, Int<2>{}, std::false_type{});
  return mt == 1 ? f(Int<1>{}, Int<1>{}, std::false_type{}) : f(Int<1>{}, Int<2>{}, std::false_type{});
}
constexpr size_t kPersistLds = 160 * 1024;
template <auto Kernel>
std::atomic<int> g_dynamic_lds_set[kMaxDevices];
bool additive_lds_fits(const dpgo_problem_s* p, int split, int mt, int na) {
  hipFuncAttributes a{};
  const int rc = dispatch_dr(p->d, p->r, [&](auto Dc, auto Rc) {
    return dispatch_persist(split, mt, true, [&](auto Sc, auto Mc, auto Ac) {
      HIPC(hipFuncGetAttributes(&a, reinterpret_cast<const void*>(
                                        &k_rtr_persist<decltype(Dc)::value, decltype(Rc)::value, decltype(Sc)::value,
                                                       decltype(Mc)::value, decltype(Ac)::value>)));
      return DPGO_OK;
    });
  });
  return rc == DPGO_OK && a.sharedSizeBytes + sizeof(double) * (size_t)p->b * p->b * na <= kPersistLds;
}
PersistGeo persist_geometry(const dpgo_problem_s* p, int free_slots, int share, bool additive) {
  if (additive) {
    const int sp = additive_split_of(p);
    if (!sp) return PersistGeo();
    PersistGeo g{sp, additive_mt_of(p), p->ml[1].n, 0};
    if (g.mt == 2 && !additive_lds_fits(p, sp, g.mt, g.wgs)) return PersistGeo();
    g.slots = g.wgs * persist_slots_per_wg(sp, 1, true);
    if (g.wgs > kPersistMax || g.slots > free_slots) return PersistGeo();
    return g;
  }
  const int env_split = options().persist_split, env_mt = options().persist_mt;
  const int cand[4][2] = {{4, 1}, {4, 2}, {1, 1}, {1, 2}};
  PersistGeo compact;
  for (auto& c : cand) {
    if (env_split && c[0] != env_split) continue;
    if (env_mt && c[1] != env_mt) continue;
    const int wgs = (pose_tiles(p->n, p->b, c[0]) + c[1] - 1) / c[1];
    const int slots = wgs * persist_slots_per_wg(c[0], c[1]);
    if (wgs > kPersistMax || slots > free_slots) continue;
    const PersistGeo g{c[0], c[1], wgs, slots};
    if ((long long)slots * std::max(1, share) <= free_slots) return g;
    if (compact.wgs == 0 || slots < compact.slots) compact = g;
  }
// ... 94 lines not shown
  std::fprintf(stderr,
               "dpgo_hip: persistent tCG: %u workgroups (%d lane groups per pose, %d tiles each)%s, %u iterations; per "
               "iteration (us): Hessian phase %.2f, all-reduce %.2f, update phase %.2f, all-reduce %.2f; per solve (us): "
               "set-up + initial statistics %.1f, first updates %.1f, retraction / trial point / rho test %.1f\n",
               p->hctrl->members, p->persist_split, p->persist_mt, p->hctrl->error ? " TIMED OUT" : "", p->hctrl->iters,
               0.01 * (double)p->hctrl->ticks[0] / it, 0.01 * (double)p->hctrl->ticks[1] / it,
               0.01 * (double)p->hctrl->ticks[2] / it, 0.01 * (double)p->hctrl->ticks[3] / it,
               0.01 * (double)p->hctrl->ticks[5], 0.01 * (double)p->hctrl->ticks[6], 0.01 * (double)p->hctrl->ticks[7]);
}

int rtr_outer_iteration(dpgo_problem_s* p, const dpgo_ropt_params* prm, const double* dinv, Counters& cnt,
                        bool poll_at_end) {
  p->gen += 1;
  const bool add = prm->precond == DPGO_PRECOND_ADDITIVE;
  const bool ml = prm->precond == DPGO_PRECOND_MULTILEVEL || add;
  p->zr_from_post = ml;
  if (add) cnt.vcycle_for_additive = true;
  auto update = [&](int first) -> int {
    if (ml) {
      CHK(launch_tcg_update(p, dinv, first, p->ml[0].x1, p->ml_omega));
      const bool early_stop = options().ml_early_stop != 0;
      return launch_ml_tail(p, p->x1, p->rr, p->z, p->pB(), p->dstate + p->cur, early_stop && !first);
    }
    return launch_tcg_update(p, dinv, first);
  };
  CHK(update(1));
  const int max_inner = prm->RTR_tCG_iterations;
  auto step = [&](int j) -> int {
    CHK(launch_tcg_hess(p, j == 0 ? 1 : 0));
    return update(0);
  };
  if (max_inner <= 0) CHK(launch_tcg_hess(p, 1));
  bool done = false;
  if (prm->tcg_poll_interval > 0) {
    const int poll = prm->tcg_poll_interval;
    int j = 0;
    while (j < max_inner) {
      const int chunk = (max_inner - j) < poll ? (max_inner - j) : poll;
      for (int c = 0; c < chunk; ++c) CHK(step(j + c));
      j += chunk;
      CHK(poll_state(p));
      if (p->hstate->tcg_done || p->hstate->rtr_stop) {
        done = true;
        break;
      }
    }
  } else {
    int kAhead = ml ? 2 : 4;
    if (options().tcg_ahead > 0) kAhead = std::max(2, options().tcg_ahead);
    int enq = 0, last_j = -1;
    auto t_progress = std::chrono::steady_clock::now();
    while (true) {
      const unsigned long long w = __atomic_load_n(p->hflag.get(), __ATOMIC_ACQUIRE);
      int dev_j = 0;
      if ((unsigned)(w >> 32) == p->gen) {
        dev_j = (int)((w >> 8) & 0xFFFFFFu);
        if (w & 3ull) {
          done = true;
          if (w & 2ull) p->saw_rtr_stop = true;
          break;
        }
      }
      if (enq >= max_inner) break;
      if (dev_j != last_j) {
        last_j = dev_j;
        t_progress = std::chrono::steady_clock::now();
      }
      if (enq < dev_j + kAhead) {
        CHK(step(enq));
        enq += 1;
      } else {
        __builtin_ia32_pause();
        if (std::chrono::duration<double>(std::chrono::steady_clock::now() - t_progress).count() > 60.0) {
          HIPC(hipStreamSynchronize(p->stream));
          return fail(DPGO_ERR_HIP, "tCG progress word did not advance for 60 s");
        }
      }
    }
  }
  if (!done) CHK(launch_tcg_hess(p, 0));
  if (p->saw_rtr_stop) return DPGO_OK;
  const bool rho_exact = options().rho_exact != 0;
  CHK(launch_retract(p, p->x1, p->eta, 1.0, p->x2, p->dstate + p->cur, rho_exact ? nullptr : p->rr.get(),
                     rho_exact ? nullptr : p->g1.get()));
  CHK(launch_grad(p, p->x2, p->g2, p->S2, nullptr, p->dstate + p->cur, p->tcg_sym && outer_sym_enabled()));
  cnt.spmm += 1;
  if (rho_exact) {
    CHK(launch_hess(p, p->x1, p->S1, p->eta, p->g1, p->Hd, p->pH(), p->dstate + p->cur, 0, p->tcg_sym && outer_sym_enabled()));
    cnt.spmm += 1;
  }
  CHK(launch_rtr_update(p));
  if (poll_at_end) CHK(poll_state(p));
  return DPGO_OK;
}

constexpr int kAutoUnitsJacobi = 10, kAutoUnitsAdditive = 13, kAutoSetupUnits = 2800, kAutoMinProducts = 6;
constexpr int kAutoUnitsAdditive2 = 22;
int auto_units_jacobi(dpgo_problem_s* p) {
  const int share = std::max(1, p->persist_share);
  if (share == 1 || !p->persist) return kAutoUnitsJacobi;
  const int cap = persist_capacity(p->device), limit = cap - cap / 5;
  const PersistGeo g = persist_geometry(p, limit, share, false);
  if (g.wgs <= 0) return kAutoUnitsJacobi;
  const double part = std::max((double)g.slots / limit, 1.0 / share);
  const double two_tiles = g.mt == 2 ? (g.split == 1 ? 2.1 : 1.25) : 1.0;
  return std::max(1, (int)std::lround(kAutoUnitsJacobi * two_tiles * part * share));
}
int auto_units_additive(dpgo_problem_s* p) {
  const int share = std::max(1, p->persist_share);
  const int units = p->add_plan.tile == 2 * ml_tile(p->b, 1) ? kAutoUnitsAdditive2 : kAutoUnitsAdditive;
  if (share == 1) return units;
  const int cap = persist_capacity(p->device);
  const double part = std::max((double)(p->add_plan.na * persist_slots_per_wg(p->add_plan.split, 1, true)) / cap, 1.0 / share);
  return std::max(1, (int)std::lround(units * part * share));
}
void auto_update(dpgo_problem_s* p, const dpgo_ropt_params* prm, int used, int products) {
  const int budget = std::max(1, prm->RTR_iterations) * std::max(1, prm->RTR_tCG_iterations);
  const bool coupled = p->has_G || p->C.nnzb > 0;
  auto& a = p->auto_cost;
  a.last_used = used;
  a.last_products = products;
  if (!coupled) {
    if (!p->auto_ml && 2 * products >= budget) p->auto_ml = true;
    return;
  }
  const bool cost_rule = options().auto_cost_rule != 0;
  if (!p->auto_ml) {
    a.state = 0;
    a.uj = auto_units_jacobi(p);
    a.jac_units += (long long)kAutoUnitsJacobi * products;
    const bool binds = 2 * products >= budget;
    const bool paid = cost_rule && products >= kAutoMinProducts && a.jac_units >= ((long long)kAutoSetupUnits << a.backoff);
    if (binds || paid) {
      const bool add = cost_rule && !p->ml_user_ks && additive_available(p);
      if (add) a.ua = auto_units_additive(p);
      const bool hopeless = add && !binds && (long long)a.ua * kAutoMinProducts >= (long long)a.uj * products;
      if (hopeless) {
        a.jac_units = 0;
        a.backoff = std::min(a.backoff + 1, 6);
      } else if (binds || add) {
        p->auto_ml = true;
        if (add) {
          a.state = 1;
          a.ref = products;
          a.switches += 1;
        }
      }
    }
    return;
  }
  if (a.state == 0) {
    if (10 * products <= budget) p->auto_ml = false;
    return;
  }
  a.ua = auto_units_additive(p);
  const long long cost = (long long)a.ua * products * 100, ref = (long long)a.uj * a.ref * (a.state == 2 ? 115 : 100);
  if (cost < ref) {
    a.state = 2;
  } else {
    p->auto_ml = false;
    a.state = 0;
    a.jac_units = 0;
    a.backoff = std::min(a.backoff + 1, 6);
  }
}

int run_optimize(dpgo_problem_s* p, const dpgo_ropt_params* prm, dpgo_ropt_result* res, int phase) {
  auto t0 = std::chrono::steady_clock::now();
  Counters cnt;
  std::memset(res, 0, sizeof(*res));
  res->tCGStatus = DPGO_TCG_MAXITER;
  const bool resume = phase == RUN_END;
  if (p->hctrl && !resume) std::memset(p->hctrl, 0, sizeof(PersistCtrl));
  struct SlotGuard {
    dpgo_problem_s* p;
    bool armed;
    ~SlotGuard() {
      if (armed) persist_release(p);
    }
  } slot_guard{p, true};
  dpgo_ropt_params resolved = resume ? p->pending.resolved : *prm;
  if (!resume) {
    if (prm->precond == DPGO_PRECOND_AUTO) p->auto_decide();
    if (prm->precond == DPGO_PRECOND_AUTO)
      resolved.precond = (p->auto_ml && prm->method == DPGO_METHOD_RTR)
                             ? ((additive_available(p) && !p->ml_user_ks) ? DPGO_PRECOND_ADDITIVE : DPGO_PRECOND_MULTILEVEL)
                             : DPGO_PRECOND_BLOCK_JACOBI;
  }
  const bool is_auto = resume ? p->pending.is_auto : prm->precond == DPGO_PRECOND_AUTO;
  if (resume) t0 = p->pending.t0;
  prm = &resolved;
  const double* dinv = nullptr;
  if (resume) {
    dinv = p->pending.dinv;
  } else
  if (prm->precond == DPGO_PRECOND_BLOCK_JACOBI) {
    CHK(build_dinv(p, prm->precond_shift));
    dinv = p->dinv;
  } else if (prm->precond == DPGO_PRECOND_MULTILEVEL) {
    CHK(ml_ensure(p, prm->precond_shift));
    dinv = p->dinv;
  } else if (prm->precond == DPGO_PRECOND_ADDITIVE) {
    if (prm->method != DPGO_METHOD_RTR) return fail(DPGO_ERR_UNSUPPORTED, "the additive preconditioner exists inside the tCG loop only");
    if (!additive_split_of(p) && !additive_plan(p).split)
      return fail(DPGO_ERR_UNSUPPORTED, "additive preconditioner: block too large (at most 256 aggregates of one workgroup tile, " +
                                            std::to_string(ml_tile(p->b, 1)) + " poses" +
                                            (additive_tiles(p) == 2 ? ", or of two" : "; dpgo_problem_additive_tiles: two") + ")");
    CHK(ml_ensure(p, prm->precond_shift, true));
    dinv = p->dinv;
  } else if (prm->precond != DPGO_PRECOND_NONE) {
    return fail(DPGO_ERR_INVALID, "unknown preconditioner");
  }
  if (!resume) {
    p->loop_extra_bytes = 0;
    if (prm->precond == DPGO_PRECOND_MULTILEVEL && !p->ml.empty()) {
      const size_t nd = (size_t)p->dense.lda;
      size_t bytes = nd * nd * (size_t)(p->ml_coarse_bits / 8) / (p->ml_use_dense_sym() ? 2 : 1);
      const auto& L0 = p->ml[0];
      bytes += (size_t)L0.AP.nnzb * (sizeof(double) * p->b * p->b + sizeof(int32_t)) + sizeof(double) * (size_t)p->n * p->b * p->b;
      bytes += 3 * p->vec_bytes();
      p->loop_extra_bytes = bytes;
    }
    CHK(resolve_tcg_storage(p));
    if (prm->precond == DPGO_PRECOND_MULTILEVEL) CHK(ml_ops32_ensure(p));
  }
  const bool add = prm->precond == DPGO_PRECOND_ADDITIVE;
  const bool epochs_fit = (long long)std::max(1, prm->RTR_iterations) * (3LL * std::max(0, prm->RTR_tCG_iterations) + 4) + 1 < (1LL << 20);
  if (resume || (prm->method == DPGO_METHOD_RTR && prm->RTR_iterations != 1 && prm->tcg_poll_interval <= 0 && p->persist && epochs_fit &&
                 !p->persist_failed_once && (add || prm->precond == DPGO_PRECOND_BLOCK_JACOBI || prm->precond == DPGO_PRECOND_NONE))) {
    bool used = resume;
    if (!resume) CHK(launch_rtr_persistent(p, prm, dinv, &used, add));
    if (used) {
      if (!resume) {
        if (phase == RUN_BEGIN) {
          auto& pd = p->pending;
          pd.launched = true;
          pd.resolved = resolved;
          pd.is_auto = is_auto;
          pd.dinv = dinv;
          pd.t0 = t0;
          slot_guard.armed = false;
          return DPGO_OK;
        }
      }
      HIPC(hipStreamSynchronize(p->stream));
      persist_report(p);
      if (p->hstate->rtr_stop != kPersistPoison && !p->hctrl->error) {
        const DevState& h = *p->hstate;
        res->fInit = h.fInit;
        res->gradNormInit = h.gnInit;
        res->fOpt = h.f1;
        res->gradNormOpt = h.ngf;
        res->tCGStatus = h.outer_iter > 0 ? h.tcg_status : DPGO_TCG_MAXITER;
        res->rtr_iterations = h.outer_iter;
        res->rtr_accepted = h.n_accept;
        res->latest_step_accepted = h.accepted_last;
        res->tcg_iterations = h.n_hess;
        res->precond_used = prm->precond;
        res->spmm_count = 1 + 2 * h.outer_iter + h.n_hess;
        if (is_auto) auto_update(p, prm, prm->precond, h.n_hess);
        res->success = 1;
        res->elapsedMs = 1e3 * std::chrono::duration<double>(std::chrono::steady_clock::now() - t0).count();
        return DPGO_OK;
      }
      p->persist_failed_once = true;
      p->pctrl_dirty = true;
      persist_release(p);
      if (options().persist_verbose)
        std::fprintf(stderr, "dpgo_hip: persistent solve timed out; this handle continues with the multi-launch scheme\n");
    }
  }
  CHK(launch_grad(p, p->x1, p->g1, p->S1, nullptr, nullptr, prm->method == DPGO_METHOD_RTR && p->tcg_sym && outer_sym_enabled()));
  cnt.spmm += 1;
  CHK(launch_rtr_begin(p, prm->gradnorm_tol, prm->RTR_initial_radius, 5.0 * prm->RTR_initial_radius,
                       prm->RTR_tCG_iterations, prm->accept_tiny_decrease));
  const bool deferred = prm->method == DPGO_METHOD_RTR && prm->RTR_iterations != 1 && prm->tcg_poll_interval <= 0;
  if (!deferred) {
    CHK(poll_state(p));
    res->fInit = p->hstate->fInit;
    res->gradNormInit = p->hstate->gnInit;
  } else {
    p->hstate->rtr_stop = 0;
  }
  int n_hess_total = 0;
  int shrink_tries = 0;

  if (prm->method == DPGO_METHOD_RTR) {
    if (!p->hstate->rtr_stop) {
      if (prm->RTR_iterations == 1) {
        double radius = prm->RTR_initial_radius;
        int total_steps = 0;
        while (true) {
          shrink_tries += 1;
          p->hstate->Delta = radius;
          p->hstate->Delta_max = radius;
          p->hstate->outer_iter = 0;
          CHK(push_state(p));
          p->saw_rtr_stop = false;
          CHK(rtr_outer_iteration(p, prm, dinv, cnt, true));
          if (p->hstate->accepted_last) break;
          if (total_steps > 10) break;
          radius /= 4.0;
          total_steps++;
        }
      } else {
        const bool polling = prm->tcg_poll_interval > 0;
        p->saw_rtr_stop = false;
        for (int it = 0; it < prm->RTR_iterations; ++it) {
          CHK(rtr_outer_iteration(p, prm, dinv, cnt, polling));
          if (polling ? (p->hstate->rtr_stop != 0) : p->saw_rtr_stop) break;
          const double el = std::chrono::duration<double>(std::chrono::steady_clock::now() - t0).count();
          if (prm->time_bound_s > 0 && el > prm->time_bound_s) break;
        }
        CHK(poll_state(p));
        if (deferred) {
          res->fInit = p->hstate->fInit;
          res->gradNormInit = p->hstate->gnInit;
        }
      }
      res->tCGStatus = p->hstate->tcg_status;
      res->rtr_iterations = (prm->RTR_iterations == 1) ? shrink_tries : p->hstate->outer_iter;
      res->rtr_accepted = p->hstate->n_accept;
      res->latest_step_accepted = p->hstate->accepted_last;
      n_hess_total = p->hstate->n_hess;
    }
    res->fOpt = p->hstate->f1;
    res->gradNormOpt = p->hstate->ngf;
  } else if (prm->method == DPGO_METHOD_RGD) {
    const double* step = p->g1;
    if (prm->RGD_use_preconditioner) {
      if (prm->precond == DPGO_PRECOND_MULTILEVEL)
        CHK(launch_ml_apply(p, p->x1, p->g1, p->z));
      else
        CHK(launch_precond(p, p->x1, p->g1, dinv, p->z));
      step = p->z;
    }
    CHK(launch_retract(p, p->x1, step, -prm->RGD_stepsize, p->x2, nullptr));
    HIPC(hipMemcpyAsync(p->x1, p->x2, p->vec_bytes(), hipMemcpyDeviceToDevice, p->stream));
    CHK(launch_grad(p, p->x1, p->g1, p->S1, nullptr));
    cnt.spmm += 1;
    CHK(launch_rtr_begin(p, prm->gradnorm_tol, prm->RTR_initial_radius, 5.0 * prm->RTR_initial_radius,
                         prm->RTR_tCG_iterations, prm->accept_tiny_decrease));
    CHK(poll_state(p));
    res->fOpt = p->hstate->f1;
    res->gradNormOpt = p->hstate->ngf;
  } else {
    return fail(DPGO_ERR_INVALID, "unknown method");
  }
  res->tcg_iterations = n_hess_total;
  res->precond_used = (prm->precond == DPGO_PRECOND_ADDITIVE && cnt.vcycle_for_additive) ? DPGO_PRECOND_MULTILEVEL : prm->precond;
  if (is_auto && prm->method == DPGO_METHOD_RTR) auto_update(p, prm, res->precond_used, n_hess_total);
  res->spmm_count = cnt.spmm + n_hess_total;
  res->success = 1;
  res->elapsedMs = 1e3 * std::chrono::duration<double>(std::chrono::steady_clock::now() - t0).count();
// ... 336 lines not shown
  });
}


int dpgo_problem_eval_terms_device_many(int count, const dpgo_problem_t* handles, const double* const* X_dev,
                                        const double* const* nbr_tiles_dev, void* after_stream, double* terms) {
  if (count <= 0) return DPGO_OK;
  if (!X_dev || !terms) return fail(DPGO_ERR_INVALID, "null pointer");
  for (int k = 0; k < count; ++k)
    if (!X_dev[k]) return fail(DPGO_ERR_INVALID, "null iterate");
  return run_many(count, handles, after_stream, [&](int k) -> int {
    dpgo_problem_s* p = handles[k];
    if (nbr_tiles_dev && nbr_tiles_dev[k]) {
      if (!p->C.rowptr) return fail(DPGO_ERR_STATE, "G coupling not set");
      CHK(launch_spmm(p, p->C, nbr_tiles_dev[k], p->G0, p->G));
      p->has_G = true;
    }
    CHK(launch_grad(p, X_dev[k], nullptr, nullptr, nullptr));
    CHK(launch_rtr_begin(p, 0.0, 1.0, 1.0, 0, 0));
    CHK(poll_state(p));
    terms[3 * k + 0] = p->hstate->xqx;
    terms[3 * k + 1] = p->hstate->xg;
    terms[3 * k + 2] = p->hstate->ngf * p->hstate->ngf;
    return DPGO_OK;
  });
}


#ifdef DPGO_TIMELINE
int dpgo_debug_timeline(long long* out ) {
  HIPC(hipDeviceSynchronize());
  HIPC(hipMemcpyFromSymbol(out, HIP_SYMBOL(g_timeline), sizeof(long long) * 32));
  return DPGO_OK;
}
int dpgo_debug_timeline_tiles(long long* out ) {
  HIPC(hipDeviceSynchronize());
  HIPC(hipMemcpyFromSymbol(out, HIP_SYMBOL(g_tl_tiles), sizeof(long long) * 3 * 64));
  return DPGO_OK;
}
#endif


int dpgo_problem_persistent_info(dpgo_problem_t p, int* enabled, int* workgroups, int* last_members, int* last_iterations,
                                 int* last_layout) {
  if (!p) return fail(DPGO_ERR_INVALID, "null handle");
  if (enabled) *enabled = (p->persist && !p->persist_failed_once) ? 1 : 0;
  if (workgroups) *workgroups = p->persist_wgs;
  if (last_members) *last_members = p->hctrl ? (int)p->hctrl->members : 0;
  if (last_iterations) *last_iterations = p->hctrl ? (int)p->hctrl->iters : 0;
  if (last_layout) *last_layout = (p->hctrl && p->hctrl->members) ? p->persist_split * 16 + p->persist_mt : 0;
  return DPGO_OK;
}


int dpgo_problem_persistent_phases(dpgo_problem_t p, double us_per_iteration[4], int* iterations) {
  if (!p || !us_per_iteration) return fail(DPGO_ERR_INVALID, "null handle / pointer");
  const double it = p->hctrl ? (double)p->hctrl->ticks[4] : 0.0;
  for (int k = 0; k < 4; ++k)
    us_per_iteration[k] = (p->hctrl && it > 0.0 && p->hctrl->members) ? 0.01 * (double)p->hctrl->ticks[k] / it : 0.0;
  if (iterations) *iterations = (p->hctrl && p->hctrl->members) ? (int)p->hctrl->iters : 0;
  return DPGO_OK;
}


int dpgo_problem_set_persistent(dpgo_problem_t p, int enable) {
  if (!p) return fail(DPGO_ERR_INVALID, "null handle");
  if (enable && persist_geometry(p, persist_capacity(p->device)).wgs <= 0)
    return fail(DPGO_ERR_UNSUPPORTED, "block too large for the persistent tCG kernel (at most 2 tiles on each of 256 workgroups)");
  p->persist = enable != 0;
  if (enable) p->persist_failed_once = false;
  return DPGO_OK;
}


int dpgo_problem_tcg_kernel_info(dpgo_problem_t p, int* symmetric, int* split, int* stream_nt) {
  CHK(check_ready(p));
  CHK(resolve_tcg_storage(p));
  if (symmetric) *symmetric = p->tcg_sym ? 1 : 0;
  if (split) *split = p->tcg_sym ? 1 : p->split;
  if (stream_nt) *stream_nt = (p->stream_nt && (p->tcg_sym || p->split == 1)) ? 1 : 0;
  return DPGO_OK;
}

}
```

### dpgo_amd/lib.py

```python
from __future__ import annotations

import ctypes as C
import os
import sys
from typing import Optional

import numpy as np

_HERE = os.path.dirname(os.path.abspath(__file__))
LIB_PATH = os.environ.get("DPGO_LIB") or os.path.join(_HERE, "libdpgo_hip.so")

OK, ERR_INVALID, ERR_HIP, ERR_UNSUPPORTED, ERR_STATE = 0, 1, 2, 3, 4
METHOD_RTR, METHOD_RGD = 0, 1
PRECOND_NONE, PRECOND_BLOCK_JACOBI, PRECOND_MULTILEVEL, PRECOND_AUTO, PRECOND_ADDITIVE = 0, 1, 2, 3, 4
PRECOND_NAMES = ["none", "jacobi", "multilevel", "auto", "additive"]
ML_P_BLOCKS, ML_A_ROWPTR, ML_A_COLIDX, ML_A_VALUES, ML_DENSE_INVERSE, ML_AGG_LABELS, ML_AP_NNZB = 0, 1, 2, 3, 4, 5, 6
ML_RESTRICT_PARTIALS = 7
TCG_STATUS = ["NEGCURVTURE", "EXCREGION", "LCON", "SCON", "MAXITER"]


class DpgoError(RuntimeError):
    def __init__(self, code: int, msg: str):
        super().__init__("dpgo_hip error %d: %s" % (code, msg))
        self.code = code
# ... 36 lines not shown


class ReweightStatsC(C.Structure):
    _fields_ = [("inliers", C.c_int), ("outliers", C.c_int), ("undecided", C.c_int), ("skipped", C.c_int),
                ("max_rsq", C.c_double), ("cost", C.c_double)]


CERT_CERTIFIED, CERT_NOT_CERTIFIED, CERT_NOT_CONVERGED = 0, 1, 2
CERT_STATUS = ["CERTIFIED", "NOT_CERTIFIED", "NOT_CONVERGED"]


_P = C.c_void_p
_I = C.c_int
_D = C.c_double
_PI32 = C.POINTER(C.c_int32)
_PD = C.POINTER(C.c_double)

SIGNATURES = {
    "dpgo_version": ([], C.c_char_p),
    "dpgo_last_error": ([], C.c_char_p),
    "dpgo_device_count": ([C.POINTER(C.c_int)], _I),
    "dpgo_ropt_params_default": ([C.POINTER(RoptParamsC)], None),
    "dpgo_supported": ([_I, _I], _I),
    "dpgo_describe_options": ([C.c_char_p, _I], _I),
    "dpgo_options_reload": ([], _I),
    "dpgo_problem_describe": ([_P, C.c_char_p, _I], _I),
    "dpgo_problem_create": ([C.POINTER(_P), _I, _I, _I, _I], _I),
    "dpgo_problem_destroy": ([_P], _I),
    "dpgo_problem_set_stream": ([_P, _P], _I),
    "dpgo_problem_use_own_stream": ([_P], _I),
    "dpgo_problem_dims": ([_P, C.POINTER(_I), C.POINTER(_I), C.POINTER(_I), C.POINTER(_I)], _I),
    "dpgo_problem_set_Q_bsr": ([_P, _I, _P, _P, _P], _I),
    "dpgo_problem_set_Q_csr": ([_P, _P, _P, _P], _I),
    "dpgo_problem_update_Q_values": ([_P, _P], _I),
    "dpgo_problem_set_reweightable_edges": ([_P, _I, _P, _P, _P, _P, _P, _P, _P, _P], _I),
    "dpgo_problem_set_reweightable_edges_ex": ([_P, _I, _P, _P, _P, _P, _P, _P, _P, _P, _P, _P], _I),
    "dpgo_problem_gnc_reweight_device": ([_P, _P, _P, _D, _D, _D, _I, C.POINTER(C.c_int * 3), C.POINTER(_D)], _I),
    "dpgo_problem_gnc_reweight": ([_P, _P, _D, _D, _D, _I, C.POINTER(C.c_int * 3), C.POINTER(_D)], _I),
    "dpgo_robust_cost_default": ([C.POINTER(RobustCostC)], None),
    "dpgo_problem_robust_reweight_device": ([_P, _P, _P, C.POINTER(RobustCostC), _D, _I, C.POINTER(ReweightStatsC)], _I),
    "dpgo_problem_robust_reweight": ([_P, _P, C.POINTER(RobustCostC), _D, _I, C.POINTER(ReweightStatsC)], _I),
    "dpgo_problem_set_edge_weights": ([_P, _P], _I),
    "dpgo_problem_get_edge_weights": ([_P, _P, _P], _I),
    "dpgo_problem_get_Q_values": ([_P, _P], _I),
    "dpgo_multilevel_default_ks": ([_I, _I, _P, C.POINTER(_I)], _I),
    "dpgo_multilevel_graph_aggregates": ([_I, _P, _P, _I, _P, _P, C.POINTER(_I)], _I),
    "dpgo_multilevel_merged_aggregates": ([_I, _P, _P, _I, _I, _P, _P, C.POINTER(_I)], _I),
    "dpgo_problem_additive_plan": ([_P] + [C.POINTER(_I)] * 6, _I),
    "dpgo_problem_additive_tiles": ([_P, C.POINTER(_I)], _I),
    "dpgo_problem_setup_multilevel": ([_P, _I, _P, _D, _D], _I),
    "dpgo_problem_multilevel_info": ([_P, C.POINTER(_I), _P, _P, _P], _I),
    "dpgo_problem_multilevel_get": ([_P, _I, _I, _P], _I),
    "dpgo_dense_spd_inverse": ([_I, _P, _P, _I, _I], _I),
    "dpgo_problem_multilevel_path": ([_P, C.POINTER(_I)], _I),
    "dpgo_problem_multilevel_coarse_bits": ([_P, C.POINTER(_I)], _I),
    "dpgo_problem_multilevel_operator_bits": ([_P, C.POINTER(_I), C.POINTER(_I)], _I),
    "dpgo_problem_auto_state": ([_P, C.POINTER(_I)], _I),
    "dpgo_problem_auto_info": ([_P, C.POINTER(_I), C.POINTER(C.c_longlong)] + [C.POINTER(_I)] * 5, _I),
    "dpgo_auto_rule_constants": ([C.POINTER(_I)] * 4, _I),
    "dpgo_problem_set_G": ([_P, _P], _I),
    "dpgo_problem_set_G_device": ([_P, _P], _I),
    "dpgo_problem_set_G_coupling": ([_P, _I, _I, _P, _P, _P, _P], _I),
    "dpgo_problem_update_G_from_neighbors_device": ([_P, _P], _I),
    "dpgo_problem_f": ([_P, _P, C.POINTER(_D)], _I),
    "dpgo_problem_euc_grad": ([_P, _P, _P], _I),
    "dpgo_problem_euc_hess": ([_P, _P, _P], _I),
    "dpgo_problem_rie_grad": ([_P, _P, _P], _I),
    "dpgo_problem_rie_grad_norm": ([_P, _P, C.POINTER(_D)], _I),
    "dpgo_problem_rie_hess": ([_P, _P, _P, _P], _I),
    "dpgo_problem_precondition": ([_P, _I, _D, _P, _P, _P], _I),
    "dpgo_optimize": ([_P, C.POINTER(RoptParamsC), _P, _P, C.POINTER(RoptResultC)], _I),
    "dpgo_optimize_device": ([_P, C.POINTER(RoptParamsC), _P, C.POINTER(RoptResultC)], _I),
    "dpgo_warning_count": ([], _I),
    "dpgo_optimize_device_begin": ([_P, C.POINTER(RoptParamsC), _P, _P], _I),
    "dpgo_optimize_device_end": ([_P, C.POINTER(RoptResultC)], _I),
    "dpgo_optimize_device_many": ([_I, _P, C.POINTER(RoptParamsC), _P, _P, _P, _P], _I),
    "dpgo_problem_eval_terms_device_many": ([_I, _P, _P, _P, _P, _P], _I),
    "dpgo_spmm_device": ([_P, _P, _P, _I], _I),
    "dpgo_problem_eval_device": ([_P, _P, C.POINTER(_D), C.POINTER(_D)], _I),
    "dpgo_problem_eval_terms_device": ([_P, _P, C.POINTER(_D), C.POINTER(_D), C.POINTER(_D)], _I),
    "dpgo_bench_spmm": ([_P, _I, _I, C.POINTER(_D)], _I),
    "dpgo_problem_set_spmm_variant": ([_P, _I, C.POINTER(_I)], _I),
    "dpgo_problem_tcg_kernel_info": ([_P, C.POINTER(_I), C.POINTER(_I), C.POINTER(_I)], _I),
    "dpgo_bench_spmm_rotating": ([_P, _I, _I, _I, C.POINTER(_D), C.POINTER(_D)], _I),
    "dpgo_bench_hess_rotating": ([_P, _I, _I, _I, C.POINTER(_D)], _I),
    "dpgo_bench_hess": ([_P, _I, _I, C.POINTER(_D)], _I),
    "dpgo_bench_solve": ([_P, C.POINTER(RoptParamsC), _P, _I, _I, C.POINTER(_D), C.POINTER(_D), C.POINTER(_I)], _I),
    "dpgo_bench_iteration_kernels": ([_P, _I, _I, _P], _I),
    "dpgo_manifold_project": ([_I, _I, _I, _P, _P, _I], _I),
    "dpgo_manifold_tangent_project": ([_I, _I, _I, _P, _P, _P, _I], _I),
    "dpgo_manifold_retract": ([_I, _I, _I, _P, _P, _D, _P, _I], _I),
    "dpgo_manifold_project_device": ([_I, _I, _I, _P, _P, _P], _I),
    "dpgo_round_trajectory": ([_I, _I, _I, _P, _P, _P, _I], _I),
    "dpgo_round_trajectory_device": ([_I, _I, _I, _P, _P, _P, _P], _I),
    "dpgo_gather_tiles_device": ([_I, _I, _P, _P, _I, _P, _P], _I),
    "dpgo_locality_order": ([_I, _P, _P, _I, _I, _P], _I),
    "dpgo_locality_order_runs": ([_I, _P, _P, _I, _I, _I, _P], _I),
    "dpgo_permute_tiles_device": ([_I, _I, _I, _P, _P, _P, _I, _P], _I),
    "dpgo_exchange_plan_create": ([C.POINTER(_P), _I, _I, _I, _P, _P, _P, _P, _I], _I),
    "dpgo_exchange_plan_run": ([_P, _P], _I),
    "dpgo_exchange_plan_destroy": ([_P], _I),
    "dpgo_flags_write_device": ([_I, _P, _P, _P], _I),
    "dpgo_flags_wait_device": ([_I, _P, _P, _I, _P], _I),
    "dpgo_flags_wait_device_checked": ([_I, _P, _P, C.c_longlong, _P, _P], _I),
    "dpgo_max_translation_distance_device": ([_I, _I, _I, _P, _P, _P, C.POINTER(_D), _P], _I),
    "dpgo_axpby_project_device": ([_I, _I, _I, _D, _P, _D, _P, _D, _P, _I, _P, _P], _I),
    "dpgo_problem_set_persistent": ([_P, _I], _I),
    "dpgo_problem_persistent_info": ([_P, C.POINTER(_I), C.POINTER(_I), C.POINTER(_I), C.POINTER(_I), C.POINTER(_I)], _I),
    "dpgo_problem_persistent_phases": ([_P, _P, C.POINTER(_I)], _I),
    "dpgo_chordal_initialization": ([_I, _I, _I, _P, _P, _P, _P, _P, _P, _D, _I, _P, _P, _I], _I),
    "dpgo_odometry_initialization": ([_I, _I, _I, _P, _P, _P, _P, _P], _I),
    "dpgo_device_malloc": ([C.POINTER(_P), C.c_size_t, _I], _I),
    "dpgo_device_free": ([_P], _I),
    "dpgo_device_memcpy": ([_P, _P, C.c_size_t, _I, _P], _I),
    "dpgo_device_synchronize": ([_P], _I),
    "dpgo_comm_unique_id": ([_P], _I),
    "dpgo_comm_create": ([C.POINTER(_P), _I, _I, _P, _I], _I),
    "dpgo_comm_destroy": ([_P], _I),
    "dpgo_comm_info": ([_P, C.POINTER(_I), C.POINTER(_I)], _I),
    "dpgo_comm_exchange": ([_P, _I, _P, _P, _P, _I, _P, _P, _P, _P], _I),
    "dpgo_comm_allreduce": ([_P, _P, _I, _I, _P], _I),
    "dpgo_comm_broadcast": ([_P, _P, _I, _I, _P], _I),
    "dpgo_build_Q_bsr": ([_I, _I, _I, _I, _P, _P, _P, _P, _P, _P, _P, _P, _P, _I, _P, _D, _D,
                          C.POINTER(_I), _P, _P, _P], _I),
    "dpgo_build_G_coupling": ([_I, _I, _I, _I, _P, _P, _P, _P, _P, _P, _P, _P, _P, _P,
                               C.POINTER(_I), _P, _P, _P], _I),
    "dpgo_debug_reduction_primitives": ([_I, _I, _I, _P, _P, _P, _P, _P], _I),
    "dpgo_debug_live_allocations": ([C.POINTER(C.c_longlong), C.POINTER(C.c_longlong)], _I),
    "dpgo_certify_params_default": ([C.POINTER(CertifyParamsC)], None),
    "dpgo_problem_certify": ([_P, _P, C.POINTER(CertifyParamsC), C.POINTER(CertifyResultC), _P], _I),
    "dpgo_problem_certify_device": ([_P, _P, C.POINTER(CertifyParamsC), C.POINTER(CertifyResultC), _P], _I),
    "dpgo_problem_certificate_apply": ([_P, _P, _P, _P], _I),
    "dpgo_certify_escape_device": ([_P, _I, _P, _P, _D, _P, C.POINTER(_D)], _I),
}

_lib: Optional[C.CDLL] = None


def load() -> C.CDLL:
    global _lib
    if _lib is not None:
        return _lib
    if not os.path.exists(LIB_PATH):
        raise ImportError(
            "dpgo_amd: %s not found -- build it with `python -c 'import __graft_entry__ as g; g.build()'` "
            "or `make -C dpgo_amd/csrc`.  There is no CPU fallback." % LIB_PATH)
    if "torch" not in sys.modules:
        try:
            import torch
        except ImportError:
            pass
    lib = C.CDLL(LIB_PATH)
    for name, (argtypes, restype) in SIGNATURES.items():
        fn = getattr(lib, name)
        fn.argtypes = argtypes
        fn.restype = restype
    _lib = lib
    return lib


def check(rc: int) -> None:
    if rc != OK:
        raise DpgoError(rc, load().dpgo_last_error().decode("utf-8", "replace"))


def ptr(a) -> Optional[int]:
# ... 30 lines not shown
```

### dpgo_amd/solver.py

```python
from __future__ import annotations

import ctypes as C
from dataclasses import dataclass
from typing import Dict, Optional, Tuple

import numpy as np

from . import lib as L
from .measurements import RelativeSEMeasurements


@dataclass
class ROptParameters:
    method: str = "RTR"
    verbose: bool = False
    gradnorm_tol: float = 1e-2
    RGD_stepsize: float = 1e-3
    RGD_use_preconditioner: bool = True
    RTR_iterations: int = 3
    RTR_tCG_iterations: int = 50
    RTR_initial_radius: float = 100.0
    precond: str = "auto"
    precond_shift: float = 1e-1
    accept_tiny_decrease: bool = True
# ... 342 lines not shown
                self._g_obj = False
        else:
            G = pg.linearMatrix()
            if self._g_obj is not G:
                L.check(self._lib.dpgo_problem_set_G(self._h, L.ptr(G)))
                self._g_obj = G

    def _in(self, X, what="Y"):
        return _colmajor(X, self.relaxation_rank(), self._N(), what)

    def _out(self):
        return np.empty((self.relaxation_rank(), self._N()), order="F")

    def f(self, Y) -> float:
        Yc = self._in(Y)
        out = C.c_double(0.0)
        L.check(self._lib.dpgo_problem_f(self._h, L.ptr(Yc), C.byref(out)))
        return out.value

    def EucGrad(self, X) -> np.ndarray:
        Xc, o = self._in(X), self._out()
        L.check(self._lib.dpgo_problem_euc_grad(self._h, L.ptr(Xc), L.ptr(o)))
        return o

    def EucHessianEta(self, X, V) -> np.ndarray:
        Vc, o = self._in(V, "V"), self._out()
        L.check(self._lib.dpgo_problem_euc_hess(self._h, L.ptr(Vc), L.ptr(o)))
        return o

    def RieHessianEta(self, X, V) -> np.ndarray:
        Xc, Vc, o = self._in(X), self._in(V, "V"), self._out()
        L.check(self._lib.dpgo_problem_rie_hess(self._h, L.ptr(Xc), L.ptr(Vc), L.ptr(o)))
        return o

    def PreConditioner(self, X, inVec, precond: str = "multilevel", shift: float = 1e-1) -> np.ndarray:
        Xc, Vc, o = self._in(X), self._in(inVec, "inVec"), self._out()
        pc = {"jacobi": L.PRECOND_BLOCK_JACOBI, "none": L.PRECOND_NONE, "multilevel": L.PRECOND_MULTILEVEL,
              "auto": L.PRECOND_AUTO}[precond]
        L.check(self._lib.dpgo_problem_precondition(self._h, pc, shift, L.ptr(Xc), L.ptr(Vc), L.ptr(o)))
        return o

    def RieGrad(self, Y) -> np.ndarray:
        Yc, o = self._in(Y), self._out()
        L.check(self._lib.dpgo_problem_rie_grad(self._h, L.ptr(Yc), L.ptr(o)))
        return o

    def RieGradNorm(self, Y) -> float:
        Yc = self._in(Y)
        out = C.c_double(0.0)
        L.check(self._lib.dpgo_problem_rie_grad_norm(self._h, L.ptr(Yc), C.byref(out)))
        return out.value

    def certify(self, X, witness: bool = True, **params):
        from .certificate import certify
        return certify(self, X, witness=witness, **params)

    def certificateApply(self, X, V) -> np.ndarray:
        from .certificate import certificate_apply
        return certificate_apply(self, X, V)

    def setStream(self, hip_stream: Optional[int]) -> None:
        L.check(self._lib.dpgo_problem_set_stream(self._h, hip_stream or None))

    def useOwnStream(self) -> None:
        L.check(self._lib.dpgo_problem_use_own_stream(self._h))

    def setCouplingFromPoseGraph(self) -> list:
        slots, rowptr, colidx, vals, G0 = self.pose_graph_.couplingMatrix()
        L.check(self._lib.dpgo_problem_set_G_coupling(self._h, len(slots), len(colidx), L.ptr(rowptr),
                                                      L.ptr(colidx) if len(colidx) else None,
                                                      L.ptr(vals) if len(colidx) else None, L.ptr(G0)))
        return slots

    def updateLinearMatrixFromNeighbors(self, nbr_tiles_dev) -> None:
        L.check(self._lib.dpgo_problem_update_G_from_neighbors_device(self._h, L.ptr(nbr_tiles_dev)))
        self._g_obj = None

    def setPersistent(self, enable: bool = True) -> None:
        L.check(self._lib.dpgo_problem_set_persistent(self._h, int(enable)))

    def tcgKernelInfo(self) -> dict:
        v = [C.c_int(0) for _ in range(3)]
        L.check(self._lib.dpgo_problem_tcg_kernel_info(self._h, *[C.byref(x) for x in v]))
        return dict(symmetric=bool(v[0].value), split=v[1].value, stream_nt=bool(v[2].value))

    def persistentInfo(self) -> dict:
        v = [C.c_int(0) for _ in range(5)]
        L.check(self._lib.dpgo_problem_persistent_info(self._h, *[C.byref(x) for x in v]))
        out = dict(zip(("enabled", "workgroups", "last_members", "last_iterations"), (x.value for x in v[:4])))
        out["last_split"], out["last_tiles"] = v[4].value // 16, v[4].value % 16
        return out

    def persistentPhases(self) -> dict:
        v = (C.c_double * 4)()
        it = C.c_int(0)
        L.check(self._lib.dpgo_problem_persistent_phases(self._h, v, C.byref(it)))
        return dict(hessian=v[0], reduce_after_hessian=v[1], update=v[2], reduce_after_update=v[3], iterations=it.value)

    def multilevelPath(self) -> dict:
        v = C.c_int(0)
        L.check(self._lib.dpgo_problem_multilevel_path(self._h, C.byref(v)))
        return dict(ap=bool(v.value & 1), packed_dense=bool(v.value & 2))

    def multilevelCoarseBits(self, bits=None) -> int:
        v = C.c_int(-1 if bits is None else int(bits))
        L.check(self._lib.dpgo_problem_multilevel_coarse_bits(self._h, C.byref(v)))
        return int(v.value)

    def multilevelOperatorBits(self, bits=None) -> dict:
        v, act = C.c_int(-1 if bits is None else int(bits)), C.c_int(0)
        L.check(self._lib.dpgo_problem_multilevel_operator_bits(self._h, C.byref(v), C.byref(act)))
        return dict(bits=int(v.value), active=bool(act.value & 1), vectors=bool(act.value & 2), dense=bool(act.value & 4))

    def setupMultilevel(self, ks=None, omega: float = 0.7, shift: float = 1e-1, coarse_bits=None) -> dict:
        self.refresh()
        if coarse_bits is not None:
            self.multilevelCoarseBits(coarse_bits)
        ks = L.i32(ks if ks is not None else [])
        L.check(self._lib.dpgo_problem_setup_multilevel(self._h, len(ks), L.ptr(ks) if len(ks) else None,
                                                        float(omega), float(shift)))
        return self.multilevelInfo()

    def setSpmmVariant(self, variant: str = "auto") -> str:
        self.refresh()
        names = {"auto": 0, "plain": 1, "symmetric": 2}
        if variant not in names:
            raise ValueError("variant must be one of %s" % sorted(names))
        v = C.c_int(0)
        L.check(self._lib.dpgo_problem_set_spmm_variant(self._h, names[variant], C.byref(v)))
        return "symmetric" if v.value == 2 else "plain"

    def describe(self) -> str:
        buf = C.create_string_buffer(32768)
        L.check(self._lib.dpgo_problem_describe(self._h, buf, len(buf)))
        return buf.value.decode("utf-8", "replace")

    def autoState(self, use_multilevel=None) -> bool:
        v = C.c_int(-1 if use_multilevel is None else (-2 if use_multilevel == "reset" else int(bool(use_multilevel))))
        L.check(self._lib.dpgo_problem_auto_state(self._h, C.byref(v)))
        return bool(v.value)

    def autoInfo(self) -> dict:
        st, ref, sw, bo, uj, ua = (C.c_int(0) for _ in range(6))
        units = C.c_longlong(0)
        L.check(self._lib.dpgo_problem_auto_info(self._h, C.byref(st), C.byref(units), C.byref(ref), C.byref(sw), C.byref(bo),
                                                 C.byref(uj), C.byref(ua)))
        k = [C.c_int(0) for _ in range(4)]
        L.check(self._lib.dpgo_auto_rule_constants(*[C.byref(x) for x in k]))
        return dict(state=("jacobi", "trial", "additive")[st.value], jacobi_units=int(units.value),
                    reference_products=ref.value, switches=sw.value, backoff=bo.value,
                    units_jacobi=uj.value, units_additive=ua.value, units_jacobi_alone=k[0].value,
                    units_additive_alone=k[1].value, setup_units=k[2].value, min_products=k[3].value)

    def multilevelInfo(self) -> dict:
        cap = 16
        nl = C.c_int(cap)
        sizes, ks, nnzb = (np.zeros(cap, dtype=np.int32) for _ in range(3))
        L.check(self._lib.dpgo_problem_multilevel_info(self._h, C.byref(nl), L.ptr(sizes), L.ptr(ks), L.ptr(nnzb)))
        n = nl.value
        kk = [int(v) for v in ks[:n - 1]] + ([int(ks[n - 1])] if n >= 2 and ks[n - 1] < 0 else [])
        return dict(sizes=[int(v) for v in sizes[:n]], ks=kk, nnzb=[int(v) for v in nnzb[:n]])

    def additivePlan(self) -> dict:
        v = [C.c_int(0) for _ in range(6)]
        L.check(self._lib.dpgo_problem_additive_plan(self._h, *[C.byref(x) for x in v]))
        keys = ("lane_groups", "tile", "growth", "merge_cap", "aggregates", "graph")
        out = {k: int(x.value) for k, x in zip(keys, v)}
# ... 245 lines not shown
```

### include/dpgo_hip.h

```cpp
#ifndef DPGO_HIP_H
#define DPGO_HIP_H

#include <stddef.h>
#include <stdint.h>

#ifdef __cplusplus
extern "C" {
#endif

#define DPGO_OK 0
#define DPGO_ERR_INVALID 1
#define DPGO_ERR_HIP 2
#define DPGO_ERR_UNSUPPORTED 3
#define DPGO_ERR_STATE 4

#define DPGO_METHOD_RTR 0
#define DPGO_METHOD_RGD 1

#define DPGO_PRECOND_NONE 0
#define DPGO_PRECOND_BLOCK_JACOBI 1
#define DPGO_PRECOND_MULTILEVEL 2
#define DPGO_PRECOND_AUTO 3
#define DPGO_PRECOND_ADDITIVE 4

// ... 81 lines not shown
  double tls_threshold;
} dpgo_robust_cost;
typedef struct dpgo_reweight_stats {
  int inliers, outliers, undecided, skipped;
  double max_rsq, cost;
} dpgo_reweight_stats;
void dpgo_robust_cost_default(dpgo_robust_cost* c);
int dpgo_problem_robust_reweight_device(dpgo_problem_t h, const double* X_dev, const double* nbr_tiles_dev,
                                        const dpgo_robust_cost* cost, double w_tol, int update,
                                        dpgo_reweight_stats* stats);
int dpgo_problem_robust_reweight(dpgo_problem_t h, const double* X_host, const dpgo_robust_cost* cost, double w_tol,
                                 int update, dpgo_reweight_stats* stats);

int dpgo_problem_get_Q_values(dpgo_problem_t h, double* vals_host);
#define DPGO_ML_P_BLOCKS 0
#define DPGO_ML_A_ROWPTR 1
#define DPGO_ML_A_COLIDX 2
#define DPGO_ML_A_VALUES 3
#define DPGO_ML_DENSE_INVERSE 4
#define DPGO_ML_AGG_LABELS 5
#define DPGO_ML_AP_NNZB 6
#define DPGO_ML_RESTRICT_PARTIALS 7
int dpgo_multilevel_default_ks(int n, int d, int* ks, int* nks);
int dpgo_multilevel_graph_aggregates(int n, const int32_t* rowptr, const int32_t* colidx, int max_size, int32_t* label,
                                     int32_t* parent, int* n_aggregates);
int dpgo_multilevel_merged_aggregates(int n, const int32_t* rowptr, const int32_t* colidx, int max_size, int merge_cap,
                                      int32_t* label, int32_t* parent, int* n_aggregates);
int dpgo_problem_additive_plan(dpgo_problem_t h, int* lane_groups, int* tile, int* growth, int* merge_cap, int* aggregates,
                               int* graph);
int dpgo_problem_additive_tiles(dpgo_problem_t h, int* tiles);
int dpgo_problem_setup_multilevel(dpgo_problem_t h, int nks, const int* ks, double omega, double shift);
int dpgo_problem_multilevel_info(dpgo_problem_t h, int* nlevels, int* sizes, int* ks, int* nnzb);
int dpgo_problem_multilevel_get(dpgo_problem_t h, int level, int what, void* out_host);
#define DPGO_ML_PATH_AP 1
#define DPGO_ML_PATH_PACKED_DENSE 2
int dpgo_problem_multilevel_path(dpgo_problem_t h, int* flags);
int dpgo_problem_multilevel_coarse_bits(dpgo_problem_t h, int* bits);
int dpgo_problem_multilevel_operator_bits(dpgo_problem_t h, int* bits, int* active);
int dpgo_problem_auto_state(dpgo_problem_t h, int* use_multilevel);
int dpgo_problem_auto_info(dpgo_problem_t h, int* state, long long* jacobi_units, int* reference_products, int* switches,
                           int* backoff, int* units_jacobi, int* units_additive);
int dpgo_auto_rule_constants(int* units_jacobi, int* units_additive, int* setup_units, int* min_products);
int dpgo_dense_spd_inverse(int N, const double* A_host, double* Ainv_host, int device, int use_mfma);

int dpgo_problem_set_G(dpgo_problem_t h, const double* G_host);
int dpgo_problem_set_G_device(dpgo_problem_t h, const double* G_dev);
int dpgo_problem_set_G_coupling(dpgo_problem_t h, int ncols, int nnzb, const int32_t* rowptr,
                                const int32_t* colidx, const double* vals, const double* G0_host);
int dpgo_problem_update_G_from_neighbors_device(dpgo_problem_t h, const double* nbr_tiles_dev);

int dpgo_problem_f(dpgo_problem_t h, const double* X, double* f);
int dpgo_problem_euc_grad(dpgo_problem_t h, const double* X, double* EG);
int dpgo_problem_euc_hess(dpgo_problem_t h, const double* V, double* HV);
int dpgo_problem_rie_grad(dpgo_problem_t h, const double* X, double* RG);
int dpgo_problem_rie_grad_norm(dpgo_problem_t h, const double* X, double* gn);
int dpgo_problem_rie_hess(dpgo_problem_t h, const double* X, const double* V, double* HV);
int dpgo_problem_precondition(dpgo_problem_t h, int precond, double shift, const double* X,
                              const double* V, double* Z);


int dpgo_optimize(dpgo_problem_t h, const dpgo_ropt_params* params, const double* X0, double* Xopt,
                  dpgo_ropt_result* result);
int dpgo_optimize_device(dpgo_problem_t h, const dpgo_ropt_params* params, double* X_dev,
                         dpgo_ropt_result* result);
int dpgo_warning_count(void);
int dpgo_optimize_device_begin(dpgo_problem_t h, const dpgo_ropt_params* params, double* X_dev,
                               const double* nbr_tiles_dev);
int dpgo_optimize_device_end(dpgo_problem_t h, dpgo_ropt_result* result);

int dpgo_optimize_device_many(int count, const dpgo_problem_t* handles, const dpgo_ropt_params* params,
                              double* const* X_dev, const double* const* nbr_tiles_dev, void* after_stream,
                              dpgo_ropt_result* results);
int dpgo_problem_eval_terms_device_many(int count, const dpgo_problem_t* handles, const double* const* X_dev,
                                        const double* const* nbr_tiles_dev, void* after_stream, double* terms);

int dpgo_spmm_device(dpgo_problem_t h, const double* V_dev, double* OUT_dev, int add_G);
int dpgo_problem_eval_device(dpgo_problem_t h, const double* X_dev, double* f, double* gradnorm);
int dpgo_problem_eval_terms_device(dpgo_problem_t h, const double* X_dev, double* xqx, double* xg, double* g2);
#define DPGO_SPMM_AUTO 0
#define DPGO_SPMM_PLAIN 1
#define DPGO_SPMM_SYMMETRIC 2
int dpgo_problem_set_spmm_variant(dpgo_problem_t h, int variant, int* in_use);
int dpgo_problem_tcg_kernel_info(dpgo_problem_t h, int* symmetric, int* split, int* stream_nt);
int dpgo_bench_spmm(dpgo_problem_t h, int reps, int warmup, double* avg_ms);
int dpgo_bench_spmm_rotating(dpgo_problem_t h, int nsets, int reps, int warmup, double* avg_ms, double* set_bytes);
int dpgo_bench_hess(dpgo_problem_t h, int reps, int warmup, double* avg_ms);
int dpgo_bench_solve(dpgo_problem_t h, const dpgo_ropt_params* params, const double* X0_dev, int reps, int warmup,
                     double* avg_ms, double* avg_products, int* persistent);
int dpgo_bench_hess_rotating(dpgo_problem_t h, int nsets, int reps, int warmup, double* avg_ms);
int dpgo_bench_iteration_kernels(dpgo_problem_t h, int reps, int warmup, double out_ms[5]);

int dpgo_debug_reduction_primitives(int workgroups, int pay, int steps, const double* in_dev, const double* pay_in_dev,
                                    double* sums_dev, double* pay_out_dev, double* rows_out_dev);

int dpgo_debug_live_allocations(long long* buffers, long long* bytes);

int dpgo_problem_set_persistent(dpgo_problem_t h, int enable);
int dpgo_problem_persistent_info(dpgo_problem_t h, int* enabled, int* workgroups, int* last_members,
                                 int* last_iterations, int* last_layout);
int dpgo_problem_persistent_phases(dpgo_problem_t h, double us_per_iteration[4], int* iterations);

int dpgo_locality_order(int n, const int32_t* rowptr, const int32_t* colidx, int nparts, int align, int32_t* new_index);
int dpgo_locality_order_runs(int n, const int32_t* rowptr, const int32_t* colidx, int nparts, int align, int run,
                             int32_t* new_index);
int dpgo_permute_tiles_device(int r, int d, int n, const int32_t* new_index_dev, const double* in_dev, double* out_dev,
                              int forward, void* stream);

int dpgo_chordal_initialization(int d, int n, int m, const int32_t* p1, const int32_t* p2, const double* R,
                                const double* t, const double* kappa, const double* tau, double tol, int max_iter,
                                double* T_host, int iters_out[2], int device);
int dpgo_odometry_initialization(int d, int n, int m, const int32_t* p1, const int32_t* p2, const double* R,
                                 const double* t, double* T_host);

#define DPGO_COPY_H2D 0
#define DPGO_COPY_D2H 1
#define DPGO_COPY_D2D 2
int dpgo_device_malloc(void** out, size_t bytes, int device);
int dpgo_device_free(void* p);
int dpgo_device_memcpy(void* dst, const void* src, size_t bytes, int kind, void* stream);
int dpgo_device_synchronize(void* stream);

#define DPGO_COMM_ID_BYTES 128
#define DPGO_COMM_SUM 0
#define DPGO_COMM_MAX 1
typedef struct dpgo_comm_s* dpgo_comm_t;
int dpgo_comm_unique_id(char id[DPGO_COMM_ID_BYTES]);
int dpgo_comm_create(dpgo_comm_t* out, int nranks, int rank, const char id[DPGO_COMM_ID_BYTES], int device);
int dpgo_comm_destroy(dpgo_comm_t c);
int dpgo_comm_info(dpgo_comm_t c, int* nranks, int* rank);
int dpgo_comm_exchange(dpgo_comm_t c, int nsend, const int* send_peer, const double* const* send_dev,
                       const int* send_count, int nrecv, const int* recv_peer, double* const* recv_dev,
                       const int* recv_count, void* stream);
int dpgo_comm_allreduce(dpgo_comm_t c, double* buf_dev, int count, int op, void* stream);
int dpgo_comm_broadcast(dpgo_comm_t c, double* buf_dev, int count, int root, void* stream);

int dpgo_manifold_project(int r, int d, int n, const double* M, double* out, int device);
int dpgo_manifold_tangent_project(int r, int d, int n, const double* X, const double* V, double* out,
                                  int device);
int dpgo_manifold_retract(int r, int d, int n, const double* X, const double* eta, double scale,
                          double* out, int device);
int dpgo_manifold_project_device(int r, int d, int n, const double* M_dev, double* out_dev, void* stream);
int dpgo_round_trajectory(int r, int d, int n, const double* X_host, const double* anchor_host, double* T_host,
                          int device);
int dpgo_round_trajectory_device(int r, int d, int n, const double* X_dev, const double* anchor_host, double* T_dev,
                                 void* stream);

typedef struct dpgo_exchange_plan_s* dpgo_exchange_plan_t;
int dpgo_exchange_plan_create(dpgo_exchange_plan_t* out, int r, int d, int nmsg, const double* const* src_dev,
                              const int32_t* const* idx_dev, const int* count, double* const* dst_dev, int device);
int dpgo_exchange_plan_run(dpgo_exchange_plan_t plan, void* stream);
int dpgo_exchange_plan_destroy(dpgo_exchange_plan_t plan);
int dpgo_flags_write_device(int n, unsigned long long* const* words_dev, const unsigned long long* values, void* stream);
int dpgo_flags_wait_device(int n, unsigned long long* const* words_dev, const unsigned long long* values, int timeout_ms,
                           void* stream);
int dpgo_flags_wait_device_checked(int n, unsigned long long* const* words_dev, const unsigned long long* values,
                                   long long timeout_ms, unsigned long long* err_word, void* stream);

int dpgo_max_translation_distance_device(int r, int d, int n, const double* X_dev, const double* Xprev_dev,
                                         double* out_dev, double* out_host, void* stream);
int dpgo_gather_tiles_device(int r, int d, const double* src_dev, const int32_t* idx_dev, int count,
                             double* dst_dev, void* stream);
int dpgo_axpby_project_device(int r, int d, int n, double a, const double* A_dev, double b,
                              const double* B_dev, double c, const double* C_dev, int project,
                              double* out_dev, void* stream);

int dpgo_build_Q_bsr(int my_id, int d, int n, int m, const int32_t* r1, const int32_t* p1, const int32_t* r2,
// ... 50 lines not shown
```

Before: 263.7 it/s.

## Defer tCG eta accumulation to retraction via a ring of stored directions

The multi-launch tCG keeps each search direction in its own ring slot and records the step coefficients, instead of reading and writing eta (eta += alpha*delta) in every update kernel. k_retract rebuilds eta once as a linear combination of the stored directions. This removes one read and one write of eta, plus a read of delta, from every tCG update pass. In exchange it adds memory for the ring (tCG-iterations pose vectors) and a retraction that reads every stored direction.

Result: faster. 272.8 it/s, median of 6 (+3.5%).

```diff
diff --git a/dpgo_amd/csrc/agents.hip b/dpgo_amd/csrc/agents.hip
--- a/dpgo_amd/csrc/agents.hip
+++ b/dpgo_amd/csrc/agents.hip
@@ -739,7 +739,8 @@
   HIPC(hipMemcpy(x, X, vb, hipMemcpyHostToDevice));
   HIPC(hipMemcpy(v, eta, vb, hipMemcpyHostToDevice));
   CHK(dispatch_dr(d, r, [&](auto D, auto R) {
-    return launch(k_retract<D, R>, tiles_grid(d, n), 0, nullptr, x, v, scale, o, nullptr, n, nullptr, nullptr, nullptr);
+    return launch(k_retract<D, R>, tiles_grid(d, n), 0, nullptr, x, v, scale, o, nullptr, n, nullptr, nullptr, nullptr, nullptr,
+                  nullptr, nullptr);
   }));
   HIPC(hipGetLastError());
   HIPC(hipMemcpy(out, o, vb, hipMemcpyDeviceToHost));
diff --git a/dpgo_amd/csrc/host.h b/dpgo_amd/csrc/host.h
--- a/dpgo_amd/csrc/host.h
+++ b/dpgo_amd/csrc/host.h
@@ -182,6 +182,8 @@
   X(stream_nt,         "DPGO_STREAM_NT",         -1,  "non-temporal single-use operands in the tCG-step kernels: 0 / 1")             \
   X(outer_sym,         "DPGO_OUTER_SYM",          1,  "outer RTR iteration (k_grad / k_hess) reads the symmetric copy when tCG does") \
   X(rho_exact,         "DPGO_RHO_EXACT",          0,  "rho test from a fresh H eta (k_hess, one more pass over Q) instead of tCG's residual: reference path") \
+  X(tcg_dirs,          "DPGO_TCG_DIRS",           1,  "multi-launch tCG keeps its directions and k_retract sums eta once (0: eta += alpha delta every iteration: reference path)") \
+  X(tcg_dirs_max_mb,   "DPGO_TCG_DIRS_MAX_MB", 4096,  "largest direction ring (RTR_tCG_iterations pose vectors) a solve may hold; beyond it the solve runs the reference path") \
   X(tile_walk,         "DPGO_TILE_WALK",          1,  "symmetric-storage kernels walk each XCD's tiles breadth-first over the tile graph (0: index order)") \
   X(tcg_ahead,         "DPGO_TCG_AHEAD",          0,  "iterations the just-in-time feed stays ahead (0: 2 multilevel / 4 otherwise)") \
   X(grid_update,       "DPGO_GRID_UPDATE",        0,  "launch cap of k_tcg_update (0: resident count)")                              \
@@ -265,6 +267,9 @@
   double dinv_shift = -1.0;
   DevBuf<double> x1_buf, x2, g1, g2, eta, delta, Hd, rr, z, S1, S2;
   double* x1 = nullptr;
+  DevBuf<double> dirs, dirs_coef;
+  int dirs_cap = 0;
+  bool dirs_on = false;
   struct MlLevel {
     int n = 0;
     int k = 0;
@@ -592,7 +597,7 @@
 int launch_hess(dpgo_problem_s* p, const double* X, const double* S, const double* V, const double* Gdot,
                 double* HV, double* partials, const DevState* st, int check_tcg, bool sym = false);
 int launch_retract(dpgo_problem_s* p, const double* X, const double* eta, double scale, double* X2,
-                   const DevState* st, const double* rho_r = nullptr, const double* rho_g = nullptr);
+                   const DevState* st, const double* rho_r = nullptr, const double* rho_g = nullptr, bool from_dirs = false);
 int launch_rtr_update(dpgo_problem_s* p);
 int launch_precond(dpgo_problem_s* p, const double* X, const double* V, const double* dinv, double* Z);
 int launch_rtr_begin(dpgo_problem_s* p, double tol, double Delta0, double Dmax, int max_inner, int tiny);
@@ -641,6 +646,7 @@
 int launch_tcg_hess_with(dpgo_problem_s* p, const DevState* sin, DevState* sout, int first, unsigned long long* hflag,
                          unsigned gen);
 int resolve_tcg_storage(dpgo_problem_s* p);
+int tcg_dirs_ensure(dpgo_problem_s* p, int max_inner, bool may_alloc = true);
 int persist_capacity(int device);
 bool persist_reserve(dpgo_problem_s* p, int slots, int limit);
 void persist_release(dpgo_problem_s* p);
diff --git a/dpgo_amd/csrc/kernels/manifold.h b/dpgo_amd/csrc/kernels/manifold.h
--- a/dpgo_amd/csrc/kernels/manifold.h
+++ b/dpgo_amd/csrc/kernels/manifold.h
@@ -43,30 +43,99 @@
   }
 }
 
-template <int D, int R, bool RHO = false>
+constexpr int kDirsInFlight = 4;
+template <int D, int R, bool RHO = false, bool DEF = false>
 __global__ __launch_bounds__(kBlock) void k_retract(const double* __restrict__ X, const double* __restrict__ eta,
                                                     double scale, double* __restrict__ X2,
                                                     const DevState* __restrict__ st, int n,
                                                     const double* __restrict__ r, const double* __restrict__ g,
-                                                    double* __restrict__ partials) {
+                                                    double* __restrict__ partials, const double* __restrict__ dirs,
+                                                    const double* __restrict__ coef, double* __restrict__ eta_out) {
   using GEO = Geo<D, R>;
-  __shared__ double sm[kWaves][GEO::G][GEO::T];
+  using SPN = Span<D, R, 1>;
+  constexpr bool kSpanSum = DEF && SPN::kOk;
+  __shared__ __attribute__((aligned(16))) double sm[kWaves][GEO::G][GEO::T];
   __shared__ double red[kWaves * kNP];
   if (st && st->rtr_stop) return;
   const LaneId L = lane_id<D>();
   const int ntiles = (n + GEO::P - 1) / GEO::P;
   [[maybe_unused]] double part[2] = {0.0, 0.0};
+  [[maybe_unused]] int ndirs = 0;
+  if constexpr (DEF) ndirs = (int)coef[0];
+  [[maybe_unused]] const size_t slot = (size_t)n * GEO::T;
   const TileIter ti_ = tile_iter(ntiles);
   for (int tile = ti_.first; tile < ti_.last; tile += ti_.step) {
     const int i = tile * GEO::P + L.wave * GEO::G + L.g;
     const bool ok = (L.g < GEO::G) && (i < n);
     const size_t off = (size_t)i * GEO::T + L.c * R;
     double* as = ok ? &sm[L.wave][L.g][0] : nullptr;
+    if constexpr (kSpanSum) {
+      const int lane = threadIdx.x & 63;
+      const int p0 = tile * GEO::P + L.wave * GEO::G;
+      const int npose = (n - p0) < GEO::G ? (n - p0) : GEO::G;
+      const int valid = npose > 0 ? npose * GEO::T : 0;
+      const size_t base = (size_t)p0 * GEO::T;
+      dbl2 e2[SPN::NIT];
+#pragma unroll
+      for (int it = 0; it < SPN::NIT; ++it) e2[it].x = e2[it].y = 0.0;
+      for (int k0 = 0; k0 < ndirs; k0 += kDirsInFlight) {
+        dbl2 dv[kDirsInFlight][SPN::NIT];
+#pragma unroll
+        for (int q = 0; q < kDirsInFlight; ++q)
+          if (k0 + q < ndirs) {
+            const dbl2* d2 = reinterpret_cast<const dbl2*>(dirs + (size_t)(k0 + q) * slot + base);
+#pragma unroll
+            for (int it = 0; it < SPN::NIT; ++it)
+              if (2 * (lane + 64 * it) < valid) dv[q][it] = ld_stream<1>(d2 + lane + 64 * it);
+          }
+#pragma unroll
+        for (int q = 0; q < kDirsInFlight; ++q)
+          if (k0 + q < ndirs) {
+            const double c = coef[1 + k0 + q];
+#pragma unroll
+            for (int it = 0; it < SPN::NIT; ++it)
+              if (2 * (lane + 64 * it) < valid) {
+                e2[it].x = fma(c, dv[q][it].x, e2[it].x);
+                e2[it].y = fma(c, dv[q][it].y, e2[it].y);
+              }
+          }
+      }
+#pragma unroll
+      for (int it = 0; it < SPN::NIT; ++it) {
+        const int pc = lane + 64 * it;
+        if (2 * pc < valid) {
+          reinterpret_cast<dbl2*>(&sm[L.wave][0][0])[pc] = e2[it];
+          if (eta_out) st_stream<1>(reinterpret_cast<dbl2*>(eta_out + base) + pc, e2[it]);
+        }
+      }
+      wave_sync();
+    }
     double a[R];
     if (ok) {
       double x[R], e[R];
       load_col<R>(X + off, x);
-      load_col<R>(eta + off, e);
+      if constexpr (kSpanSum) {
+        load_col<R>(as + L.c * R, e);
+      } else if constexpr (DEF) {
+#pragma unroll
+        for (int k = 0; k < R; ++k) e[k] = 0.0;
+        for (int k0 = 0; k0 < ndirs; k0 += kDirsInFlight) {
+          double dl[kDirsInFlight][R];
+#pragma unroll
+          for (int q = 0; q < kDirsInFlight; ++q)
+            if (k0 + q < ndirs) load_col<R>(dirs + (size_t)(k0 + q) * slot + off, dl[q]);
+#pragma unroll
+          for (int q = 0; q < kDirsInFlight; ++q)
+            if (k0 + q < ndirs) {
+              const double c = coef[1 + k0 + q];
+#pragma unroll
+              for (int k = 0; k < R; ++k) e[k] = fma(c, dl[q][k], e[k]);
+            }
+        }
+        if (eta_out) store_col<R>(eta_out + off, e);
+      } else {
+        load_col<R>(eta + off, e);
+      }
       if constexpr (RHO) {
         double rc[R], gc[R];
         load_col<R>(r + off, rc);
diff --git a/dpgo_amd/csrc/kernels/tcg.h b/dpgo_amd/csrc/kernels/tcg.h
--- a/dpgo_amd/csrc/kernels/tcg.h
+++ b/dpgo_amd/csrc/kernels/tcg.h
@@ -74,7 +74,19 @@
   return 0;
 }
 
-template <int D, int R, int SPLIT>
+template <int DEF>
+__device__ __forceinline__ void tcg_store_coef(double* __restrict__ coef, const DevState& st, int mode, double alpha, double tau) {
+  if constexpr (DEF) {
+    if (mode == 2) {
+      coef[0] = 0.0;
+    } else {
+      coef[1 + st.tcg_j] = (mode == 1) ? tau : alpha;
+      coef[0] = (double)(st.tcg_j + 1);
+    }
+  }
+}
+
+template <int D, int R, int SPLIT, int DEF = 0>
 __global__ __launch_bounds__(kBlock, DPGO_LB_HESS) void k_tcg_hess(BsrDev Q, const double* __restrict__ X,
                                                      const double* __restrict__ S, const double* __restrict__ z,
                                                      double* __restrict__ delta, double* __restrict__ Hd,
@@ -102,6 +114,9 @@
     publish_progress(hflag, gen, st);
   }
   if (!go) return;
+  double* dout = delta;
+  if constexpr (DEF) dout = delta + (size_t)(first ? 0 : st.tcg_j) * ((size_t)n * GEO::T);
+  const double* din = (DEF && !first) ? dout - (size_t)n * GEO::T : dout;
 
   const LaneId L = lane_id<D, SPLIT>();
   const int ntiles = (n + GEO::P - 1) / GEO::P;
@@ -125,7 +140,7 @@
         for (int a = 0; a < D; ++a) srow[a] = S[(size_t)i * D * D + L.c * D + a];
       }
       if (!first) {
-        load_col<R>(delta + off, dl);
+        load_col<R>(din + off, dl);
         load_col<R>(Hd + off, hd);
       }
     }
@@ -164,7 +179,7 @@
       }
 #pragma unroll
       for (int a = 0; a < R; ++a) part[0] = fma(dl[a], hd[a], part[0]);
-      store_col<R>(delta + off, dl);
+      store_col<R>(dout + off, dl);
       store_col<R>(Hd + off, hd);
     }
     wave_sync();
@@ -172,7 +187,7 @@
   store_partials<1>(part, pout, red);
 }
 
-template <int D, int R, int SPLIT, int NTS = 0>
+template <int D, int R, int SPLIT, int NTS = 0, int DEF = 0>
 __global__ __launch_bounds__(kBlock) void k_tcg_hess_span(BsrDev Q, const double* __restrict__ X,
                                                           const double* __restrict__ S, const double* __restrict__ z,
                                                           double* __restrict__ delta, double* __restrict__ Hd,
@@ -198,6 +213,8 @@
   double srow[D];
   int p0 = 0, valid = 0, i = 0;
   bool okp = false, ok = false;
+  const double* din = DEF ? nullptr : delta;
+  double* dout = delta;
   auto prefetch = [&](int tile) {
     p0 = tile * GEO::P + L.wave * GEO::G;
     const int npose = (n - p0) < GEO::G ? (n - p0) : GEO::G;
@@ -209,7 +226,6 @@
     const size_t base = (size_t)p0 * GEO::T;
     const dbl2* X2 = reinterpret_cast<const dbl2*>(X + base);
     const dbl2* z2 = reinterpret_cast<const dbl2*>(z + base);
-    const dbl2* d2 = reinterpret_cast<const dbl2*>(delta + base);
     const dbl2* h2 = reinterpret_cast<const dbl2*>(Hd + base);
 #pragma unroll
     for (int it = 0; it < SPN::NIT; ++it) {
@@ -218,7 +234,7 @@
         xv[it] = ld_stream<NTS>(X2 + pc);
         zv[it] = z2[pc];
         if (!first) {
-          dv[it] = ld_stream<NTS>(d2 + pc);
+          if (!DEF || din) dv[it] = ld_stream<NTS>(reinterpret_cast<const dbl2*>(din + base) + pc);
           hv[it] = ld_stream<NTS>(h2 + pc);
         }
       }
@@ -255,6 +271,20 @@
   }
   if (!go) return;
   DPGO_STAMP(0, 2);
+  if constexpr (DEF) {
+    dout = delta + (size_t)(first ? 0 : st.tcg_j) * ((size_t)n * GEO::T);
+    if (!first) {
+      din = dout - (size_t)n * GEO::T;
+      if (have) {
+        const dbl2* d2 = reinterpret_cast<const dbl2*>(din + (size_t)p0 * GEO::T);
+#pragma unroll
+        for (int it = 0; it < SPN::NIT; ++it) {
+          const int pc = lane + 64 * it;
+          if (2 * pc < valid) dv[it] = ld_stream<NTS>(d2 + pc);
+        }
+      }
+    }
+  }
 
   double part[1] = {0.0};
   while (have) {
@@ -291,7 +321,7 @@
     wave_sync();
     {
       const size_t base = (size_t)p0 * GEO::T;
-      dbl2* d2 = reinterpret_cast<dbl2*>(delta + base);
+      dbl2* d2 = reinterpret_cast<dbl2*>(dout + base);
       dbl2* h2 = reinterpret_cast<dbl2*>(Hd + base);
 #pragma unroll
       for (int it = 0; it < SPN::NIT; ++it) {
@@ -328,7 +358,7 @@
   DPGO_COMMIT(0);
 }
 
-template <int D, int R, int NTS>
+template <int D, int R, int NTS, int DEF = 0>
 __global__ __launch_bounds__(kBlock) __attribute__((amdgpu_waves_per_eu(DPGO_SYM_WAVES, DPGO_SYM_WAVES))) void k_tcg_hess_sym(BsrSymDev Q, const double* __restrict__ X,
                                                           const double* __restrict__ S, const double* __restrict__ z,
                                                           double* __restrict__ delta, double* __restrict__ Hd,
@@ -406,6 +436,9 @@
     publish_progress(hflag, gen, st);
   }
   if (!go) return;
+  double* dout = delta;
+  if constexpr (DEF) dout = delta + (size_t)(first ? 0 : st.tcg_j) * ((size_t)n * GEO::T);
+  const double* din = (DEF && !first) ? dout - (size_t)n * GEO::T : dout;
   DPGO_STAMP(0, 2);
   DPGO_STAMP_ENTRY;
   DPGO_STAMP_AT(1);
@@ -430,7 +463,7 @@
     dbl2 dv[SPN::NIT], hv[SPN::NIT];
     if (!first) {
       const size_t base = (size_t)p0 * GEO::T;
-      const dbl2* d2 = reinterpret_cast<const dbl2*>(delta + base);
+      const dbl2* d2 = reinterpret_cast<const dbl2*>(din + base);
       const dbl2* h2 = reinterpret_cast<const dbl2*>(Hd + base);
 #pragma unroll
       for (int it = 0; it < SPN::NIT; ++it) {
@@ -465,7 +498,7 @@
     DPGO_STAMP_TILE(4);
     {
       const size_t base = (size_t)p0 * GEO::T;
-      dbl2* d2 = reinterpret_cast<dbl2*>(delta + base);
+      dbl2* d2 = reinterpret_cast<dbl2*>(dout + base);
       dbl2* h2 = reinterpret_cast<dbl2*>(Hd + base);
 #pragma unroll
       for (int it = 0; it < SPN::NIT; ++it) {
@@ -512,7 +545,7 @@
 #ifndef DPGO_UPDATE_WAVES_ML
 #define DPGO_UPDATE_WAVES_ML 3
 #endif
-template <int D, int R, int ML = 0>
+template <int D, int R, int ML = 0, int DEF = 0>
 __global__ __launch_bounds__(kBlock)
     __attribute__((amdgpu_waves_per_eu(ML ? DPGO_UPDATE_WAVES_ML : (DPGO_UPDATE_WAVES ? DPGO_UPDATE_WAVES : 1),
                                        ML ? DPGO_UPDATE_WAVES_ML : (DPGO_UPDATE_WAVES ? DPGO_UPDATE_WAVES : 8))))
@@ -525,7 +558,8 @@
                                                             double* __restrict__ pout, const DevState* __restrict__ sin,
                                                             DevState* __restrict__ sout, int first, int n,
                                                             unsigned long long* hflag, unsigned gen,
-                                                            double ml_omega, float* __restrict__ z32 = nullptr) {
+                                                            double ml_omega, double* __restrict__ coef,
+                                                            float* __restrict__ z32 = nullptr) {
   using GEO = Geo<D, R>;
   using SPN = Span<D, R, 1>;
   __shared__ __attribute__((aligned(16))) double sm[kWaves][4][GEO::G][GEO::T];
@@ -553,8 +587,8 @@
     const size_t base = (size_t)p0 * GEO::T;
     const dbl2* X2 = reinterpret_cast<const dbl2*>(X + base);
     const dbl2* g2 = reinterpret_cast<const dbl2*>(g + base);
-    const dbl2* e2 = reinterpret_cast<const dbl2*>(eta + base);
-    const dbl2* d2 = reinterpret_cast<const dbl2*>(delta + base);
+    [[maybe_unused]] const dbl2* e2 = reinterpret_cast<const dbl2*>(eta + base);
+    [[maybe_unused]] const dbl2* d2 = reinterpret_cast<const dbl2*>(delta + base);
     const dbl2* h2 = reinterpret_cast<const dbl2*>(Hd + base);
     const dbl2* r2 = reinterpret_cast<const dbl2*>(r + base);
 #pragma unroll
@@ -565,8 +599,10 @@
         if (first) {
           rv[it] = g2[pc];
         } else {
-          ev[it] = e2[pc];
-          dv[it] = d2[pc];
+          if constexpr (!DEF) {
+            ev[it] = e2[pc];
+            dv[it] = d2[pc];
+          }
           hv[it] = h2[pc];
           rv[it] = r2[pc];
         }
@@ -599,6 +635,7 @@
   const int mode = tcg_update_prologue(st, pin, nb_in, first, red, alpha, tau, &praw);
   if (blockIdx.x == 0 && threadIdx.x == 0) {
     store_state(sout, st);
+    tcg_store_coef<DEF>(coef, st, mode, alpha, tau);
     publish_progress(hflag, gen, st);
   }
 
@@ -606,19 +643,22 @@
   double part[2] = {0.0, 0.0};
   while (have) {
     const size_t base = (size_t)p0 * GEO::T;
-    dbl2* eta2 = reinterpret_cast<dbl2*>(eta + base);
+    [[maybe_unused]] dbl2* eta2 = reinterpret_cast<dbl2*>(eta + base);
     if (mode == 1) {
       dbl2* r2 = reinterpret_cast<dbl2*>(r + base);
 #pragma unroll
       for (int it = 0; it < SPN::NIT; ++it) {
         const int pc = lane + 64 * it;
         if (2 * pc < valid) {
-          dbl2 e = ev[it], rr = rv[it];
-          e.x = fma(tau, dv[it].x, e.x);
-          e.y = fma(tau, dv[it].y, e.y);
+          dbl2 rr = rv[it];
+          if constexpr (!DEF) {
+            dbl2 e = ev[it];
+            e.x = fma(tau, dv[it].x, e.x);
+            e.y = fma(tau, dv[it].y, e.y);
+            eta2[pc] = e;
+          }
           rr.x = fma(tau, hv[it].x, rr.x);
           rr.y = fma(tau, hv[it].y, rr.y);
-          eta2[pc] = e;
           r2[pc] = rr;
         }
       }
@@ -631,17 +671,21 @@
           if (!ml_mode) reinterpret_cast<dbl2*>(ys)[pc] = xv[it];
           dbl2 rr = rv[it];
           if (mode == 2) {
-            dbl2 zero;
-            zero.x = 0.0;
-            zero.y = 0.0;
-            eta2[pc] = zero;
+            if constexpr (!DEF) {
+              dbl2 zero;
+              zero.x = 0.0;
+              zero.y = 0.0;
+              eta2[pc] = zero;
+            }
           } else {
-            dbl2 e = ev[it];
-            e.x = fma(alpha, dv[it].x, e.x);
-            e.y = fma(alpha, dv[it].y, e.y);
+            if constexpr (!DEF) {
+              dbl2 e = ev[it];
+              e.x = fma(alpha, dv[it].x, e.x);
+              e.y = fma(alpha, dv[it].y, e.y);
+              eta2[pc] = e;
+            }
             rr.x = fma(alpha, hv[it].x, rr.x);
             rr.y = fma(alpha, hv[it].y, rr.y);
-            eta2[pc] = e;
           }
           r2[pc] = rr;
           reinterpret_cast<dbl2*>(rs)[pc] = rr;
@@ -706,7 +750,7 @@
   DPGO_COMMIT(1);
 }
 
-template <int D, int R>
+template <int D, int R, int DEF = 0>
 __global__ __launch_bounds__(kBlock, DPGO_LB_UPDATE) void k_tcg_update(const double* __restrict__ X, const double* __restrict__ g,
                                                        const double* __restrict__ dinv,
                                                        const double* __restrict__ delta,
@@ -715,7 +759,8 @@
                                                        const double* __restrict__ pin, int nb_in,
                                                        double* __restrict__ pout, const DevState* __restrict__ sin,
                                                        DevState* __restrict__ sout, int first, int n,
-                                                       unsigned long long* hflag, unsigned gen, double ml_omega) {
+                                                       unsigned long long* hflag, unsigned gen, double ml_omega,
+                                                       double* __restrict__ coef) {
   using GEO = Geo<D, R>;
   __shared__ __attribute__((aligned(16))) double sm[kWaves][3][GEO::G][GEO::T];
   __shared__ double red[kWaves * kNP];
@@ -733,6 +778,7 @@
   const int mode = tcg_update_prologue(st, pin, nb_in, first, red, alpha, tau);
   if (blockIdx.x == 0 && threadIdx.x == 0) {
     store_state(sout, st);
+    tcg_store_coef<DEF>(coef, st, mode, alpha, tau);
     publish_progress(hflag, gen, st);
   }
 
@@ -746,17 +792,19 @@
     const size_t off = (size_t)i * GEO::T + L.c * R;
     if (mode == 1) {
       if (ok) {
-        double e[R], dl[R], hd[R], rr[R];
-        load_col<R>(eta + off, e);
-        load_col<R>(delta + off, dl);
+        double hd[R], rr[R];
+        if constexpr (!DEF) {
+          double e[R], dl[R];
+          load_col<R>(eta + off, e);
+          load_col<R>(delta + off, dl);
+#pragma unroll
+          for (int a = 0; a < R; ++a) e[a] = fma(tau, dl[a], e[a]);
+          store_col<R>(eta + off, e);
+        }
         load_col<R>(Hd + off, hd);
         load_col<R>(r + off, rr);
 #pragma unroll
-        for (int a = 0; a < R; ++a) {
-          e[a] = fma(tau, dl[a], e[a]);
-          rr[a] = fma(tau, hd[a], rr[a]);
-        }
-        store_col<R>(eta + off, e);
+        for (int a = 0; a < R; ++a) rr[a] = fma(tau, hd[a], rr[a]);
         store_col<R>(r + off, rr);
       }
       continue;
@@ -773,22 +821,26 @@
       }
       if (mode == 2) {
         load_col<R>(g + off, rr);
-        double e[R];
-#pragma unroll
-        for (int a = 0; a < R; ++a) e[a] = 0.0;
-        store_col<R>(eta + off, e);
+        if constexpr (!DEF) {
+          double e[R];
+#pragma unroll
+          for (int a = 0; a < R; ++a) e[a] = 0.0;
+          store_col<R>(eta + off, e);
+        }
       } else {
-        double e[R], dl[R], hd[R];
-        load_col<R>(eta + off, e);
-        load_col<R>(delta + off, dl);
+        double hd[R];
+        if constexpr (!DEF) {
+          double e[R], dl[R];
+          load_col<R>(eta + off, e);
+          load_col<R>(delta + off, dl);
+#pragma unroll
+          for (int a = 0; a < R; ++a) e[a] = fma(alpha, dl[a], e[a]);
+          store_col<R>(eta + off, e);
+        }
         load_col<R>(Hd + off, hd);
         load_col<R>(r + off, rr);
 #pragma unroll
-        for (int a = 0; a < R; ++a) {
-          e[a] = fma(alpha, dl[a], e[a]);
-          rr[a] = fma(alpha, hd[a], rr[a]);
-        }
-        store_col<R>(eta + off, e);
+        for (int a = 0; a < R; ++a) rr[a] = fma(alpha, hd[a], rr[a]);
       }
       store_col<R>(r + off, rr);
 #pragma unroll
diff --git a/dpgo_amd/csrc/problem.hip b/dpgo_amd/csrc/problem.hip
--- a/dpgo_amd/csrc/problem.hip
+++ b/dpgo_amd/csrc/problem.hip
@@ -255,7 +255,7 @@
 }
 
 int launch_retract(dpgo_problem_s* p, const double* X, const double* eta, double scale, double* X2,
-                   const DevState* st, const double* rho_r, const double* rho_g) {
+                   const DevState* st, const double* rho_r, const double* rho_g, bool from_dirs) {
   int gr = std::min(pose_tiles(p->n, p->b), options().grid_retract > 0 ? options().grid_retract : kMaxGrid);
   const bool rho = rho_r && rho_g;
   if (rho) {
@@ -263,9 +263,17 @@
     gr = std::min(gr, kPartialCap);
     p->nb_hess = gr;
   }
+  if (from_dirs && (!p->dirs || !p->dirs_coef || scale != 1.0))
+    return fail(DPGO_ERR_STATE, "the retraction from kept directions is the RTR step of a solve that kept them");
   CHK(dispatch_dr(p->d, p->r, [&](auto D, auto R) {
-    if (rho) return launch(k_retract<D, R, true>, gr, 0, p->stream, X, eta, scale, X2, st, p->n, rho_r, rho_g, p->pH());
-    return launch(k_retract<D, R, false>, gr, 0, p->stream, X, eta, scale, X2, st, p->n, nullptr, nullptr, nullptr);
+    auto go = [&](auto kernel) {
+      return launch(kernel, gr, 0, p->stream, X, from_dirs ? nullptr : eta, scale, X2, st, p->n, rho ? rho_r : nullptr,
+                    rho ? rho_g : nullptr,
+                    rho ? p->pH() : nullptr, from_dirs ? p->dirs.get() : nullptr, from_dirs ? p->dirs_coef.get() : nullptr,
+                    (from_dirs && !rho) ? p->eta.get() : nullptr);
+    };
+    if (from_dirs) return rho ? go(k_retract<D, R, true, true>) : go(k_retract<D, R, false, true>);
+    return rho ? go(k_retract<D, R, true>) : go(k_retract<D, R, false>);
   }));
   HIPC(hipGetLastError());
   return DPGO_OK;
@@ -515,6 +523,10 @@
       ml_free(p);
     }
     sym_free(p);
+    p->dirs = DevBuf<double>();
+    p->dirs_coef = DevBuf<double>();
+    p->dirs_cap = 0;
+    p->dirs_on = false;
   }
   p->sym.ready = p->tcg_sym = false;
   p->ml_ready = false;
diff --git a/dpgo_amd/csrc/solve.hip b/dpgo_amd/csrc/solve.hip
--- a/dpgo_amd/csrc/solve.hip
+++ b/dpgo_amd/csrc/solve.hip
@@ -10,16 +10,19 @@
   float* z32 = (ml_omega > 0.0 && !p->ml.empty() && z_out == p->ml[0].x1 && p->ml_vec32_active()) ? p->ml[0].x1f : nullptr;
   CHK(dispatch_dr(p->d, p->r, [&](auto Dc, auto Rc) {
     constexpr int D = decltype(Dc)::value, R = decltype(Rc)::value;
+    const bool def = p->dirs_on;
     auto go = [&](auto kernel, auto... z32_arg) {
-      return launch(kernel, g, 0, p->stream, p->x1, p->g1, dinv, p->delta, p->Hd, p->eta, p->rr, zt, p->pA(), p->grid_s(),
-                    p->pB(), p->dstate + p->cur, p->dstate + (p->cur ^ 1), first, p->n, p->hflag, p->gen, ml_omega,
+      return launch(kernel, g, 0, p->stream, p->x1, p->g1, dinv, def ? nullptr : p->delta.get(), p->Hd,
+                    def ? nullptr : p->eta.get(), p->rr, zt, p->pA(), p->grid_s(), p->pB(), p->dstate + p->cur,
+                    p->dstate + (p->cur ^ 1), first, p->n, p->hflag, p->gen, ml_omega, def ? p->dirs_coef.get() : nullptr,
                     z32_arg...);
     };
     if constexpr (Span<D, R, 1>::kOk) {
+      if (def) return go(ml_mode ? k_tcg_update_span<D, R, 1, 1> : k_tcg_update_span<D, R, 0, 1>, z32);
       return go(ml_mode ? k_tcg_update_span<D, R, 1> : k_tcg_update_span<D, R, 0>, z32);
     } else {
       if (z32) return fail(DPGO_ERR_STATE, "fp32 cycle vectors need the span kernels (even pose tile size)");
-      return go(k_tcg_update<D, R>);
+      return def ? go(k_tcg_update<D, R, 1>) : go(k_tcg_update<D, R>);
     }
   }));
   HIPC(hipGetLastError());
@@ -27,23 +30,29 @@
   return DPGO_OK;
 }
 
+template <int D, int R, int DEF, class F>
+int dispatch_tcg_hess_mode(const dpgo_problem_s* p, F&& f) {
+  if constexpr (Span<D, R, 1>::kOk) {
+    if (p->tcg_sym) return f(p->stream_nt ? k_tcg_hess_sym<D, R, 1, DEF> : k_tcg_hess_sym<D, R, 0, DEF>, p->sym.dev());
+    if (p->stream_nt && p->split == 1) return f(k_tcg_hess_span<D, R, 1, 1, DEF>, p->Q.dev());
+    return dispatch_split(p->split, [&](auto Sc) { return f(k_tcg_hess_span<D, R, decltype(Sc)::value, 0, DEF>, p->Q.dev()); });
+  } else {
+    return dispatch_split(p->split, [&](auto Sc) { return f(k_tcg_hess<D, R, decltype(Sc)::value, DEF>, p->Q.dev()); });
+  }
+}
 template <int D, int R, class F>
 int dispatch_tcg_hess(const dpgo_problem_s* p, F&& f) {
-  if constexpr (Span<D, R, 1>::kOk) {
-    if (p->tcg_sym) return f(p->stream_nt ? k_tcg_hess_sym<D, R, 1> : k_tcg_hess_sym<D, R, 0>, p->sym.dev());
-    if (p->stream_nt && p->split == 1) return f(k_tcg_hess_span<D, R, 1, 1>, p->Q.dev());
-    return dispatch_split(p->split, [&](auto Sc) { return f(k_tcg_hess_span<D, R, decltype(Sc)::value>, p->Q.dev()); });
-  } else {
-    return dispatch_split(p->split, [&](auto Sc) { return f(k_tcg_hess<D, R, decltype(Sc)::value>, p->Q.dev()); });
-  }
+  return p->dirs_on ? dispatch_tcg_hess_mode<D, R, 1>(p, f) : dispatch_tcg_hess_mode<D, R, 0>(p, f);
 }
 
 int launch_tcg_hess_with(dpgo_problem_s* p, const DevState* sin, DevState* sout, int first, unsigned long long* hflag,
                          unsigned gen) {
+  if (p->dirs_on && !p->dirs) return fail(DPGO_ERR_STATE, "deferred tCG launch without a direction ring");
+  double* dl = p->dirs_on ? p->dirs.get() : p->delta.get();
   CHK(dispatch_dr(p->d, p->r, [&](auto Dc, auto Rc) {
     constexpr int D = decltype(Dc)::value, R = decltype(Rc)::value;
     return dispatch_tcg_hess<D, R>(p, [&](auto kernel, const auto& Q) {
-      return launch(kernel, p->grid_s(), 0, p->stream, Q, p->x1, p->S1, p->z, p->delta, p->Hd, p->pB(), p->nb_zr(), p->pA(),
+      return launch(kernel, p->grid_s(), 0, p->stream, Q, p->x1, p->S1, p->z, dl, p->Hd, p->pB(), p->nb_zr(), p->pA(),
                     sin, sout, first, p->n, hflag, gen);
     });
   }));
@@ -72,6 +81,30 @@
   bool usable = false;
   CHK(sym_ensure(p, &usable));
   p->tcg_sym = usable;
+  return DPGO_OK;
+}
+
+int tcg_dirs_ensure(dpgo_problem_s* p, int max_inner, bool may_alloc) {
+  p->dirs_on = false;
+  if (options().tcg_dirs == 0) return DPGO_OK;
+  const int slots = std::max(1, max_inner);
+  const size_t slot = (size_t)p->n * p->T;
+  if ((double)slots * (double)slot * sizeof(double) > (double)std::max(0, options().tcg_dirs_max_mb) * 1048576.0) return DPGO_OK;
+  if (slots > p->dirs_cap || !p->dirs || !p->dirs_coef) {
+    if (!may_alloc) return DPGO_OK;
+    p->dirs = DevBuf<double>();
+    p->dirs_coef = DevBuf<double>();
+    p->dirs_cap = 0;
+    if (p->dirs.alloc((size_t)slots * slot) != DPGO_OK || p->dirs_coef.alloc((size_t)slots + 1) != DPGO_OK) {
+      (void)hipGetLastError();
+      p->dirs = DevBuf<double>();
+      p->dirs_coef = DevBuf<double>();
+      return DPGO_OK;
+    }
+    HIPC(hipMemsetAsync(p->dirs_coef, 0, sizeof(double) * ((size_t)slots + 1), p->stream));
+    p->dirs_cap = slots;
+  }
+  p->dirs_on = true;
   return DPGO_OK;
 }
 
@@ -332,7 +365,7 @@
   if (p->saw_rtr_stop) return DPGO_OK;
   const bool rho_exact = options().rho_exact != 0;
   CHK(launch_retract(p, p->x1, p->eta, 1.0, p->x2, p->dstate + p->cur, rho_exact ? nullptr : p->rr.get(),
-                     rho_exact ? nullptr : p->g1.get()));
+                     rho_exact ? nullptr : p->g1.get(), p->dirs_on));
   CHK(launch_grad(p, p->x2, p->g2, p->S2, nullptr, p->dstate + p->cur, p->tcg_sym && outer_sym_enabled()));
   cnt.spmm += 1;
   if (rho_exact) {
@@ -422,6 +455,7 @@
   res->tCGStatus = DPGO_TCG_MAXITER;
   const bool resume = phase == RUN_END;
   if (p->hctrl && !resume) std::memset(p->hctrl, 0, sizeof(PersistCtrl));
+  if (!resume) p->dirs_on = false;
   struct SlotGuard {
     dpgo_problem_s* p;
     bool armed;
@@ -520,6 +554,8 @@
         std::fprintf(stderr, "dpgo_hip: persistent solve timed out; this handle continues with the multi-launch scheme\n");
     }
   }
+  p->dirs_on = false;
+  if (prm->method == DPGO_METHOD_RTR) CHK(tcg_dirs_ensure(p, prm->RTR_tCG_iterations));
   CHK(launch_grad(p, p->x1, p->g1, p->S1, nullptr, nullptr, prm->method == DPGO_METHOD_RTR && p->tcg_sym && outer_sym_enabled()));
   cnt.spmm += 1;
   CHK(launch_rtr_begin(p, prm->gradnorm_tol, prm->RTR_initial_radius, 5.0 * prm->RTR_initial_radius,
@@ -1022,4 +1058,12 @@
   return DPGO_OK;
 }
 
-}
+
+int dpgo_problem_tcg_directions_info(dpgo_problem_t p, int* deferred, int* slots) {
+  if (!p) return fail(DPGO_ERR_INVALID, "null handle");
+  if (deferred) *deferred = p->dirs_on ? 1 : 0;
+  if (slots) *slots = p->dirs ? p->dirs_cap : 0;
+  return DPGO_OK;
+}
+
+}
diff --git a/dpgo_amd/lib.py b/dpgo_amd/lib.py
--- a/dpgo_amd/lib.py
+++ b/dpgo_amd/lib.py
@@ -142,6 +142,7 @@
     "dpgo_bench_spmm": ([_P, _I, _I, C.POINTER(_D)], _I),
     "dpgo_problem_set_spmm_variant": ([_P, _I, C.POINTER(_I)], _I),
     "dpgo_problem_tcg_kernel_info": ([_P, C.POINTER(_I), C.POINTER(_I), C.POINTER(_I)], _I),
+    "dpgo_problem_tcg_directions_info": ([_P, C.POINTER(_I), C.POINTER(_I)], _I),
     "dpgo_bench_spmm_rotating": ([_P, _I, _I, _I, C.POINTER(_D), C.POINTER(_D)], _I),
     "dpgo_bench_hess_rotating": ([_P, _I, _I, _I, C.POINTER(_D)], _I),
     "dpgo_bench_hess": ([_P, _I, _I, C.POINTER(_D)], _I),
diff --git a/dpgo_amd/solver.py b/dpgo_amd/solver.py
--- a/dpgo_amd/solver.py
+++ b/dpgo_amd/solver.py
@@ -448,7 +448,10 @@
     def tcgKernelInfo(self) -> dict:
         v = [C.c_int(0) for _ in range(3)]
         L.check(self._lib.dpgo_problem_tcg_kernel_info(self._h, *[C.byref(x) for x in v]))
-        return dict(symmetric=bool(v[0].value), split=v[1].value, stream_nt=bool(v[2].value))
+        w = [C.c_int(0) for _ in range(2)]
+        L.check(self._lib.dpgo_problem_tcg_directions_info(self._h, *[C.byref(x) for x in w]))
+        return dict(symmetric=bool(v[0].value), split=v[1].value, stream_nt=bool(v[2].value),
+                    directions=bool(w[0].value), direction_slots=w[1].value)
 
     def persistentInfo(self) -> dict:
         v = [C.c_int(0) for _ in range(5)]
diff --git a/include/dpgo_hip.h b/include/dpgo_hip.h
--- a/include/dpgo_hip.h
+++ b/include/dpgo_hip.h
@@ -187,6 +187,7 @@
 #define DPGO_SPMM_SYMMETRIC 2
 int dpgo_problem_set_spmm_variant(dpgo_problem_t h, int variant, int* in_use);
 int dpgo_problem_tcg_kernel_info(dpgo_problem_t h, int* symmetric, int* split, int* stream_nt);
+int dpgo_problem_tcg_directions_info(dpgo_problem_t h, int* deferred, int* slots);
 int dpgo_bench_spmm(dpgo_problem_t h, int reps, int warmup, double* avg_ms);
 int dpgo_bench_spmm_rotating(dpgo_problem_t h, int nsets, int reps, int warmup, double* avg_ms, double* set_bytes);
 int dpgo_bench_hess(dpgo_problem_t h, int reps, int warmup, double* avg_ms);
```
